# succinctlabs/sp1

Hardware: AMD Instinct MI355X
Metric: RISC-V cycles proved/sec (core shard prove): whole ShardProof of a full core shard of the reference's `fibonacci` guest, see config (higher is better)
Workload: dtype u32 (KoalaBear Montgomery words, exact integer arithmetic)

## Files before the change

### sp1_amd/csrc/gkr.hip

```cpp
#include <algorithm>
#include <array>
#include <chrono>
#include <cstring>
#include <memory>
#include <string>
#include <vector>

#include "device_ctx.hpp"
#include "host_par.hpp"

namespace sp1hip {
bool gkr_host_simd_available();
void gkr_host_round_sums(const uint32_t* tab, size_t stride, const uint32_t* eq, size_t eq_stride, size_t real_pairs, uint32_t out[6][4]);
void gkr_host_round_fold(const uint32_t* tab, uint32_t* out, size_t stride, size_t real_pairs, const uint32_t alpha[4]);
}
#include "round_sync.hpp"
#include "tensor_table.hpp"

namespace sp1hip {

void challenger_observe(sp1hip_challenger_t* ch, uint32_t x);
kb::Ext challenger_sample_ext(sp1hip_challenger_t* ch);
void challenger_restore(sp1hip_challenger_t* dst, const sp1hip_challenger_t* src);
void challenger_export(const sp1hip_challenger_t* ch, uint32_t* w34);
void challenger_import(sp1hip_challenger_t* ch, const uint32_t* w34);

namespace gkr {

using Ext = kb::Ext;
struct DeviceBuf : AsyncScratch {
    uint32_t* u32() const { return (uint32_t*)p; }
    Ext* ext() const { return (Ext*)p; }
};

__device__ __forceinline__ Ext ld_ext(const Ext* p, uint32_t i) {
    const q4_t v = gptr(reinterpret_cast<const q4_t*>(p))[i];
    return Ext{{v.x, v.y, v.z, v.w}};
}
__device__ __forceinline__ void st_ext(Ext* p, uint32_t i, const Ext& e) {
    const q4_t v = {e.c[0], e.c[1], e.c[2], e.c[3]};
    gptr(reinterpret_cast<q4_t*>(p))[i] = v;
}

__device__ __forceinline__ void st_ext_host(Ext* p, uint32_t i, const Ext& e) {
    uint32_t* w = reinterpret_cast<uint32_t*>(p + i);
#pragma unroll
    for (int k = 0; k < 4; k++) __hip_atomic_store(w + k, e.c[k], __ATOMIC_RELAXED, __HIP_MEMORY_SCOPE_SYSTEM);
}

__device__ __forceinline__ uint32_t wave_sum(uint32_t v) {
#pragma unroll
    for (int off = 32; off >= 1; off >>= 1) v = kb::add(v, __shfl_down(v, off, 64));
    return v;
}
template <int NS>
__device__ __forceinline__ void block_reduce_store(const Ext (&acc)[NS], uint32_t* out) {
    __shared__ uint32_t sm[4][4 * NS];
    const int lane = threadIdx.x & 63, wave = threadIdx.x >> 6;
#pragma unroll
    for (int s = 0; s < NS; s++)
#pragma unroll
        for (int k = 0; k < 4; k++) {
            const uint32_t w = wave_sum(acc[s].c[k]);
            if (lane == 0) sm[wave][4 * s + k] = w;
        }
    __syncthreads();
    if (threadIdx.x < 4 * NS) {
        uint32_t a = 0;
        for (int i = 0; i < 4; i++) a = kb::add(a, sm[i][threadIdx.x]);
        out[threadIdx.x] = a;
    }
}
template <int NS>
__global__ __launch_bounds__(256) void reduce_partials(const uint32_t* __restrict__ partials, uint32_t n, uint32_t* out) {
    Ext acc[NS];
#pragma unroll
    for (int s = 0; s < NS; s++) acc[s] = kb::ext_zero();
    for (uint32_t i = threadIdx.x; i < n; i += 256)
#pragma unroll
        for (int s = 0; s < NS; s++) {
            const uint32_t* q = partials + ((size_t)i * NS + s) * 4;
            acc[s] = kb::ext_add(acc[s], Ext{{q[0], q[1], q[2], q[3]}});
        }
    block_reduce_store<NS>(acc, out);
}

__device__ __forceinline__ uint32_t level_pos(uint32_t e, uint32_t len) {
    return (e | 511u) < len ? ((e & ~511u) | ((e & 7u) << 6) | ((e >> 3) & 63u)) : e;
}

struct IntDesc {
    const uint32_t* prog;
    const uint32_t* main;
    const uint32_t* prep;
    uint32_t rows;
    uint32_t* n_out;
    Ext* d_out;
};

// ... 442 lines not shown
            if (lane == 0) sm[wave][4 * c + k] = w;
        }
    }
    __syncthreads();
    if (threadIdx.x < 4 * OPEN_COLS) {
        const int c = threadIdx.x / 4;
        if (d.col0 + c < d.width) {
            uint32_t a = 0;
            for (int i = 0; i < 4; i++) a = kb::add(a, sm[i][threadIdx.x]);
            partials[((size_t)blockIdx.y * total_cols + d.out0 + c) * 4 + (threadIdx.x & 3)] = a;
        }
    }
}
__global__ __launch_bounds__(256) void open_sum_kernel(const uint32_t* __restrict__ partials, uint32_t n_chunks, uint32_t n_words, uint32_t* __restrict__ out) {
    __shared__ uint32_t sm[256];
    const uint32_t jl = threadIdx.x & 63u, cl = threadIdx.x >> 6, j = blockIdx.x * 64u + jl;
    uint32_t acc = 0;
    if (j < n_words)
        for (uint32_t c = cl; c < n_chunks; c += 4) acc = kb::add(acc, partials[(size_t)c * n_words + j]);
    sm[threadIdx.x] = acc;
    __syncthreads();
    if (cl == 0 && j < n_words) out[j] = kb::add(kb::add(sm[jl], sm[64 + jl]), kb::add(sm[128 + jl], sm[192 + jl]));
}

Ext operator+(const Ext& a, const Ext& b) { return kb::ext_add(a, b); }
Ext operator-(const Ext& a, const Ext& b) { return kb::ext_sub(a, b); }
Ext operator*(const Ext& a, const Ext& b) { return kb::ext_mul(a, b); }
Ext ext_c(uint32_t canonical) { return kb::ext_from_base(kb::to_monty(canonical)); }
int log2_ceil(uint64_t x) { int l = 0; while (((uint64_t)1 << l) < x) l++; return l; }

std::vector<Ext> partial_lagrange_host(const std::vector<Ext>& pt) {
    std::vector<Ext> ev{kb::ext_one()};
    for (const Ext& x : pt) {
        std::vector<Ext> nx(ev.size() * 2);
        for (size_t i = 0; i < ev.size(); i++) { const Ext pr = ev[i] * x; nx[2 * i] = ev[i] - pr; nx[2 * i + 1] = pr; }
        ev.swap(nx);
    }
    return ev;
}
Ext eval_mle_host(const std::vector<Ext>& vals, const std::vector<Ext>& pt) {
    const std::vector<Ext> eq = partial_lagrange_host(pt);
    Ext acc = kb::ext_zero();
    for (size_t i = 0; i < vals.size(); i++) acc = acc + eq[i] * vals[i];
    return acc;
}

using Poly4 = std::array<Ext, 4>;
Ext poly_eval(const Poly4& c, const Ext& x) { return ((c[3] * x + c[2]) * x + c[1]) * x + c[0]; }

Poly4 interpolate4(const Ext (&xs)[4], const Ext (&ys)[4]) {
    Poly4 res{kb::ext_zero(), kb::ext_zero(), kb::ext_zero(), kb::ext_zero()};
    Ext num[4][4], den[4];
    bool live[4];
    for (int i = 0; i < 4; i++) {
        live[i] = !kb::ext_eq(ys[i], kb::ext_zero());
        if (!live[i]) continue;
        den[i] = kb::ext_one();
        Ext cur[4] = {ys[i], kb::ext_zero(), kb::ext_zero(), kb::ext_zero()};
        int deg = 0;
        for (int j = 0; j < 4; j++) {
            if (j == i) continue;
            den[i] = den[i] * (xs[i] - xs[j]);
            Ext nxt[4] = {kb::ext_zero(), kb::ext_zero(), kb::ext_zero(), kb::ext_zero()};
            for (int k = 0; k <= deg; k++) { nxt[k + 1] = nxt[k + 1] + cur[k]; nxt[k] = nxt[k] - cur[k] * xs[j]; }
            deg++;
            for (int k = 0; k < 4; k++) cur[k] = nxt[k];
        }
        for (int k = 0; k < 4; k++) num[i][k] = cur[k];
    }
    Ext prefix[4], running = kb::ext_one();
    for (int i = 0; i < 4; i++) if (live[i]) { prefix[i] = running; running = running * den[i]; }
    Ext inv_all = kb::ext_inv(running);
    for (int i = 3; i >= 0; i--) {
        if (!live[i]) continue;
        const Ext inv = inv_all * prefix[i];
        inv_all = inv_all * den[i];
        for (int k = 0; k < 4; k++) res[k] = res[k] + num[i][k] * inv;
    }
    return res;
}

struct Bytes {
    std::vector<uint8_t> b;
    void u64(uint64_t v) { for (int i = 0; i < 8; i++) b.push_back((uint8_t)(v >> (8 * i))); }
    void felt(uint32_t m) { const uint32_t v = kb::from_monty(m); for (int i = 0; i < 4; i++) b.push_back((uint8_t)(v >> (8 * i))); }
    void ext(const Ext& e) { for (int k = 0; k < 4; k++) felt(e.c[k]); }
};

void observe_ext(sp1hip_challenger_t* ch, const Ext& e) { for (int k = 0; k < 4; k++) challenger_observe(ch, e.c[k]); }

int upload(DeviceBuf& buf, const void* src, size_t bytes, hipStream_t s, PinnedStage& stage) {
    SP1HIP_TRY(buf.alloc(std::max<size_t>(bytes, 16), s));
    return stage.upload(buf.p, src, bytes);
}

struct ChipInfo {
    std::string name;
    uint32_t rows, k, main_w, prep_w, int0;
    const uint32_t* d_main;
    const uint32_t* d_prep;
};

constexpr uint32_t MAX_TILES = 512;
uint32_t tiles_for(uint64_t threads) { return (uint32_t)std::min<uint64_t>(std::max<uint64_t>((threads + 255) / 256, 1), MAX_TILES); }
}
}

using namespace sp1hip;
using namespace sp1hip::gkr;

extern "C" {

int sp1hip_logup_gkr_prove(const sp1hip_gkr_chip_t* chips, int n_chips, int max_log_row_count, sp1hip_challenger_t* challenger,
                           uint8_t* h_proof, size_t* proof_len, sp1hip_stream_t stream) {
    SP1HIP_REQUIRE(chips && n_chips > 0 && challenger && proof_len, "bad argument");
    const int L = max_log_row_count;
    SP1HIP_REQUIRE(L >= 1 && L <= 30, "max_log_row_count out of range");
    hipStream_t s = S(stream);
    static const bool gkr_debug = env_flag("SP1HIP_GKR_DEBUG", false);
    auto t_last = std::chrono::steady_clock::now();
    auto mark = [&](const char* what) {
        if (!gkr_debug) return;
        const auto now = std::chrono::steady_clock::now();
        fprintf(stderr, "[sp1hip gkr] %-28s %8.3f ms\n", what, std::chrono::duration<double, std::milli>(now - t_last).count());
        t_last = now;
    };

    std::vector<ChipInfo> info(n_chips);
    struct ParsedInt { uint32_t is_send, kind; std::vector<uint32_t> mult; std::vector<std::vector<uint32_t>> values; };
    std::vector<ParsedInt> progs;
    size_t max_arity = 0, total_cols = 0;
    for (int c = 0; c < n_chips; c++) {
        const sp1hip_gkr_chip_t& ci = chips[c];
        SP1HIP_REQUIRE(ci.name && ci.interactions, "null chip field");
        SP1HIP_REQUIRE(ci.real_rows <= ((uint64_t)1 << L), "chip taller than 2^max_log_row_count");
        SP1HIP_REQUIRE(ci.real_rows == 0 || ci.main_width == 0 || ci.d_main, "null main trace");
        SP1HIP_REQUIRE(ci.real_rows == 0 || ci.prep_width == 0 || ci.d_prep, "null preprocessed trace");
        if (c) SP1HIP_REQUIRE(strcmp(chips[c - 1].name, ci.name) < 0, "chips must be sorted by name (BTreeSet order)");
        info[c] = ChipInfo{ci.name, (uint32_t)ci.real_rows, 0, ci.main_width, ci.prep_width, (uint32_t)progs.size(), ci.d_main, ci.d_prep};
        const uint32_t* p = ci.interactions;
        const uint32_t* end = p + ci.n_words;
        SP1HIP_REQUIRE(ci.n_words >= 1, "empty interaction program");
        const uint32_t ni = *p++;
        info[c].k = ni;
        auto vcol = [&](std::vector<uint32_t>& out) -> bool {
            if (p + 2 > end) return false;
            const uint32_t nt = p[0];
            if (p[1] >= kb::P || p + 2 + 3 * (size_t)nt > end) return false;
            out.push_back(nt);
            out.push_back(kb::to_monty(p[1]));
            p += 2;
            for (uint32_t t = 0; t < nt; t++, p += 3) {
                if (p[0] > 1 || p[2] >= kb::P) return false;
                if (p[1] >= (p[0] ? ci.main_width : ci.prep_width)) return false;
                out.push_back(p[0]); out.push_back(p[1]); out.push_back(kb::to_monty(p[2]));
            }
            return true;
        };
        for (uint32_t i = 0; i < ni; i++) {
            SP1HIP_REQUIRE(p + 3 <= end, "truncated interaction program");
            const uint32_t nv = p[2];
            SP1HIP_REQUIRE(p[0] <= 1 && p[1] < kb::P && nv < 4096, "bad interaction header");
            ParsedInt pi{p[0], p[1], {}, std::vector<std::vector<uint32_t>>(nv)};
            p += 3;
            SP1HIP_REQUIRE(vcol(pi.mult), "bad multiplicity column");
            for (uint32_t j = 0; j < nv; j++) SP1HIP_REQUIRE(vcol(pi.values[j]), "bad value column (index or weight out of range)");
            max_arity = std::max<size_t>(max_arity, nv + 1);
            progs.push_back(std::move(pi));
        }
        SP1HIP_REQUIRE(p == end, "trailing words in interaction program");
        total_cols += (size_t)ci.main_width + ci.prep_width;
    }
    const uint32_t K = (uint32_t)progs.size();
    SP1HIP_REQUIRE(K >= 1, "no interactions in the shard");
    const int niv = log2_ceil(K), beta_seed_dim = log2_ceil(max_arity);
    const uint32_t W = 1u << niv;

    size_t need = 2 * (8 + (size_t)2 * W * 16 + 24) + 8;
    for (int v = 1; v <= L - 1; v++) need += 64 + 8 + (size_t)(niv + v) * (8 + 64) + 16 + 8 + (size_t)(niv + v) * 16 + 16;
    need += 8 + (size_t)L * 16 + 8;
    for (int c = 0; c < n_chips; c++) {
        need += 8 + info[c].name.size() + 8 + (size_t)info[c].main_w * 16 + 16 + 1;
        if (info[c].prep_w) need += 8 + (size_t)info[c].prep_w * 16 + 16;
    }
    need += 4;
    if (!h_proof || *proof_len < need) {
        *proof_len = need;
        set_error("sp1hip_logup_gkr_prove: proof buffer too small, need %zu bytes", need);
        return SP1HIP_ERROR_BUFFER_TOO_SMALL;
    }

    const DeviceCtx* ctx;
    SP1HIP_TRY(get_device_ctx(&ctx));
    sp1hip_challenger_t* ch = nullptr;
    SP1HIP_TRY(sp1hip_challenger_clone(challenger, &ch));
    struct ChGuard { sp1hip_challenger_t* c; ~ChGuard() { sp1hip_challenger_free(c); } } guard{ch};

    uint32_t witness = 0;
    SP1HIP_TRY(sp1hip_challenger_grind(ch, 12, &witness, stream));
    const Ext alpha = challenger_sample_ext(ch);
    std::vector<Ext> beta_seed(beta_seed_dim);
    for (auto& b : beta_seed) b = challenger_sample_ext(ch);
    (void)challenger_sample_ext(ch);
    const std::vector<Ext> betas = partial_lagrange_host(beta_seed);

    auto rows_at = [&](uint32_t h, int l) -> uint32_t { return (uint32_t)(((uint64_t)h + (((uint64_t)1 << (L - l)) - 1)) >> (L - l)); };
    std::vector<uint32_t> int_chip(K);
    for (int c = 0; c < n_chips; c++) for (uint32_t i = 0; i < info[c].k; i++) int_chip[info[c].int0 + i] = c;
    std::vector<size_t> level_entries(L + 2, 0);
    for (int l = 1; l <= L; l++) for (uint32_t i = 0; i < K; i++) level_entries[l] += rows_at(info[int_chip[i]].rows, l);
    std::vector<DeviceBuf> lvN(L + 1), lvD(L + 1);
    for (int l = 1; l <= L; l++) {
        SP1HIP_TRY(lvN[l].alloc(std::max<size_t>(level_entries[l], 1) * (l == L ? 4 : 16), s));
        SP1HIP_TRY(lvD[l].alloc(std::max<size_t>(level_entries[l], 1) * 16, s));
    }
    std::vector<std::vector<size_t>> off(L + 1, std::vector<size_t>(K + 1, 0));
    for (int l = 1; l <= L; l++) for (uint32_t i = 0; i < K; i++) off[l][i + 1] = off[l][i] + rows_at(info[int_chip[i]].rows, l);
    auto n_ptr = [&](int l, uint32_t i) -> void* { return (char*)lvN[l].p + off[l][i] * (l == L ? 4 : 16); };
    auto d_ptr = [&](int l, uint32_t i) -> Ext* { return lvD[l].ext() + off[l][i]; };

    mark("parse + level buffers");
    const uint32_t FLAT_MAX_SLOTS = (uint32_t)env_uint("SP1HIP_GKR_FLAT_SLOTS", 65536);
    size_t n_passes_total = 0;
    for (int v = 1; v <= L - 1; v++) n_passes_total += (size_t)(v + 1) / 2 + 1;
    hipStream_t side = nullptr;
    hipEvent_t* side_ev = nullptr;
    SP1HIP_TRY(aux_stream_for(s, 2, &side, &side_ev));
    DeviceBuf d_all, d_flat;
    SP1HIP_TRY(d_all.alloc(std::max<size_t>(n_passes_total * K, 1) * sizeof(PassDesc), side));
    SP1HIP_TRY(d_flat.alloc((n_passes_total * (size_t)FLAT_MAX_SLOTS + 4) * sizeof(uint16_t), side));
    PinnedStage side_stage;
    SP1HIP_TRY(side_stage.init(side));
    PinnedStage stage;
    SP1HIP_TRY(stage.init(s));
    DeviceBuf d_progs, d_betas, d_descs;
    uint32_t max_rows = 0;
    bool fused_tree = false;
    std::vector<uint32_t> flat;
    std::vector<IntDesc> descs(K);
    {
        std::vector<size_t> poff(K);
        for (uint32_t i = 0; i < K; i++) {
            poff[i] = flat.size();
            const ParsedInt& pi = progs[i];
            Ext head = alpha + kb::ext_mul_base(betas[0], kb::to_monty(pi.kind));
            uint32_t live = 0;
            for (size_t j = 0; j < pi.values.size(); j++) {
                if (pi.values[j][0] == 0) head = head + kb::ext_mul_base(betas[1 + j], pi.values[j][1]);
                else live++;
            }
            flat.insert(flat.end(), {pi.is_send, live, head.c[0], head.c[1], head.c[2], head.c[3]});
            flat.insert(flat.end(), pi.mult.begin(), pi.mult.end());
            for (size_t j = 0; j < pi.values.size(); j++) {
                if (pi.values[j][0] == 0) continue;
                flat.push_back((uint32_t)(1 + j));
                flat.insert(flat.end(), pi.values[j].begin(), pi.values[j].end());
            }
        }
        SP1HIP_TRY(upload(d_progs, flat.data(), flat.size() * 4, s, stage));
        SP1HIP_TRY(upload(d_betas, betas.data(), betas.size() * 16, s, stage));
        for (uint32_t i = 0; i < K; i++) {
            const ChipInfo& c = info[int_chip[i]];
            descs[i] = IntDesc{d_progs.u32() + poff[i], c.d_main, c.d_prep, c.rows, (uint32_t*)n_ptr(L, i), d_ptr(L, i)};
            max_rows = std::max(max_rows, c.rows);
        }
        fused_tree = L >= 3 && env_flag("SP1HIP_GKR_FUSED", true);
        if (fused_tree) {
            std::vector<FirstDesc> fdescs(K);
            for (uint32_t i = 0; i < K; i++)
                fdescs[i] = FirstDesc{descs[i].prog, descs[i].main, descs[i].prep, descs[i].rows, descs[i].n_out, descs[i].d_out,
                                      (Ext*)n_ptr(L - 1, i), d_ptr(L - 1, i), (Ext*)n_ptr(L - 2, i), d_ptr(L - 2, i)};
            SP1HIP_TRY(upload(d_descs, fdescs.data(), fdescs.size() * sizeof(FirstDesc), s, stage));
            if (max_rows) {
                ScopedTimer t("gkr_first_layer", s);
                hipLaunchKernelGGL(first_layers_kernel, dim3(tiles_for((max_rows + 3) / 4), K), dim3(256), 0, s, (const FirstDesc*)d_descs.p,
                                   (const Ext*)d_betas.p);
                SP1HIP_LAUNCH_CHECK();
            }
        } else {
            SP1HIP_TRY(upload(d_descs, descs.data(), descs.size() * sizeof(IntDesc), s, stage));
            if (max_rows) {
                ScopedTimer t("gkr_first_layer", s);
                hipLaunchKernelGGL(first_layer_kernel, dim3(tiles_for(max_rows), K), dim3(256), 0, s, (const IntDesc*)d_descs.p,
                                   (const Ext*)d_betas.p);
                SP1HIP_LAUNCH_CHECK();
            }
        }
    }
    mark("first layer enqueued");
    DeviceBuf d_trans, d_trans2;
    {
        const int top = fused_tree ? L - 2 : L;
        std::vector<Trans2Desc> t2;
        std::vector<TransDesc> t1;
        std::vector<uint32_t> t2_mr, t1_mr;
        std::vector<int> t1_level;
        int l = top;
        if (fused_tree)
            for (; l >= 3; l -= 2) {
                uint32_t mr = 0;
                for (uint32_t i = 0; i < K; i++) {
                    const uint32_t rin = rows_at(info[int_chip[i]].rows, l);
                    t2.push_back(Trans2Desc{(const Ext*)n_ptr(l, i), d_ptr(l, i), (Ext*)n_ptr(l - 1, i), d_ptr(l - 1, i), (Ext*)n_ptr(l - 2, i), d_ptr(l - 2, i), rin});
                    mr = std::max(mr, (rin + 3) / 4);
                }
                t2_mr.push_back(mr);
            }
        for (; l >= 2; l--) {
            uint32_t mr = 0;
            for (uint32_t i = 0; i < K; i++) {
                const uint32_t rin = rows_at(info[int_chip[i]].rows, l);
                t1.push_back(TransDesc{n_ptr(l, i), d_ptr(l, i), (Ext*)n_ptr(l - 1, i), d_ptr(l - 1, i), rin});
                mr = std::max(mr, (rin + 1) / 2);
            }
            t1_mr.push_back(mr);
            t1_level.push_back(l);
        }
        if (!t2.empty()) SP1HIP_TRY(upload(d_trans2, t2.data(), t2.size() * sizeof(Trans2Desc), s, stage));
        if (!t1.empty()) SP1HIP_TRY(upload(d_trans, t1.data(), t1.size() * sizeof(TransDesc), s, stage));
        for (size_t k = 0; k < t2_mr.size(); k++) {
            if (!t2_mr[k]) continue;
            ScopedTimer t("gkr_transition", s);
            hipLaunchKernelGGL(transition2_kernel, dim3(tiles_for(t2_mr[k]), K), dim3(256), 0, s, (const Trans2Desc*)d_trans2.p + k * K);
            SP1HIP_LAUNCH_CHECK();
        }
        for (size_t k = 0; k < t1_mr.size(); k++) {
            if (!t1_mr[k]) continue;
            const TransDesc* d_t = (const TransDesc*)d_trans.p + k * K;
            ScopedTimer t("gkr_transition", s);
            if (t1_level[k] == L) hipLaunchKernelGGL(transition_kernel<true>, dim3(tiles_for(t1_mr[k]), K), dim3(256), 0, s, d_t);
            else hipLaunchKernelGGL(transition_kernel<false>, dim3(tiles_for(t1_mr[k]), K), dim3(256), 0, s, d_t);
            SP1HIP_LAUNCH_CHECK();
        }
    }
    mark("tree enqueued");
    Mailbox mb;
    SP1HIP_TRY(mb.init(s));
    struct RoundOut { Ext n0, n1, d0, d1; std::vector<Poly4> polys; Ext claimed_sum, eval; std::vector<Ext> point; };
    std::vector<RoundOut> rounds;
    DeviceBuf d_eq_int, d_T, d_TL, d_partials, scratch[2];
// ... 9 lines not shown
    std::vector<uint16_t> flat_index;
    constexpr uint32_t TARGET_TILES = 2048;
    std::vector<PassDesc> all_descs;
    all_descs.reserve(n_passes_total * K);
    const bool direct_final = (size_t)K * 16 + 4 <= MAILBOX_WORDS;
    Ext* const host_rows = reinterpret_cast<Ext*>(mb.h_slot + 4);
    for (int v = 1; v <= L - 1; v++) {
        std::vector<uint32_t> rows_in(K);
        for (uint32_t i = 0; i < K; i++) rows_in[i] = (rows_at(info[int_chip[i]].rows, v + 1) + 1) / 2;
        int cur = 0, t = v, fv = 0, pass = 0;
        std::vector<size_t> so_prev, so_next;
        for (;;) {
            const int sv = std::min(2, t - fv);
            const bool first = pass <= 1;
            if (fv > 0) { so_next.assign(K + 1, 0); for (uint32_t i = 0; i < K; i++) so_next[i + 1] = so_next[i] + ((rows_in[i] + (1u << fv) - 1) >> fv); }
            uint64_t total_slots = 0;
            auto slots_of = [&](uint32_t rin) -> uint32_t { const uint32_t ro = (rin + (1u << fv) - 1) >> fv; return ((ro + (1u << sv) - 1) >> sv) << sv; };
            for (uint32_t i = 0; i < K; i++) total_slots += slots_of(rows_in[i]);
            const bool flat = total_slots <= FLAT_MAX_SLOTS && K <= 65536;
            const uint32_t tile_size = flat ? 1u : (uint32_t)std::max<uint64_t>(256, ((total_slots + TARGET_TILES - 1) / TARGET_TILES + 255) / 256 * 256);
            const size_t flat_off = flat_index.size();
            all_descs.resize(all_descs.size() + K);
            PassDesc* out = all_descs.data() + all_descs.size() - K;
            uint32_t tile0 = 0;
            for (uint32_t i = 0; i < K; i++) {
                PassDesc& d = out[i];
                d = PassDesc{};
                d.rows_in = rows_in[i]; d.eq_int_index = i;
                if (first) { d.src[0] = n_ptr(v + 1, i); d.src[1] = d_ptr(v + 1, i); d.rows_x = rows_at(info[int_chip[i]].rows, v + 1); }
                else for (int w = 0; w < 4; w++) d.src[w] = scratch_ptr(cur ^ 1, i, w, so_prev);
                if (fv > 0) for (int w = 0; w < 4; w++)
                    d.dst[w] = (sv == 0 && direct_final) ? host_rows + 4 * so_next[i] + (size_t)w * (so_next[i + 1] - so_next[i]) : scratch_ptr(cur, i, w, so_next);
                d.tile0 = tile0;
                const uint32_t n_tiles = (slots_of(rows_in[i]) + tile_size - 1) / tile_size;
                if (flat) flat_index.insert(flat_index.end(), n_tiles, (uint16_t)i);
                tile0 += n_tiles;
            }
            if (flat) shapes.push_back(PassShape{fv, sv, first, std::max<uint32_t>((tile0 + 255) / 256, 1), tile_size, tile0, flat_off, true});
            else shapes.push_back(PassShape{fv, sv, first, std::max<uint32_t>(tile0, 1), tile_size, tile0, 0, false});
            if (fv > 0) { for (uint32_t i = 0; i < K; i++) rows_in[i] = (rows_in[i] + (1u << fv) - 1) >> fv; so_prev = so_next; cur ^= 1; }
            t -= fv;
            pass++;
            if (sv == 0) break;
            fv = sv;
        }
    }
    {
        uint32_t max_tiles = 1;
        for (auto& sh : shapes) max_tiles = std::max(max_tiles, sh.tiles);
        SP1HIP_TRY(d_partials.alloc((size_t)max_tiles * 160, s));
    }
    mark("pass descriptors planned");
    SP1HIP_REQUIRE(all_descs.size() == n_passes_total * K, "internal error: pass count");
    SP1HIP_TRY(side_stage.upload(d_all.p, all_descs.data(), all_descs.size() * sizeof(PassDesc)));
    if (flat_index.empty()) flat_index.push_back(0);
    flat_index.resize((flat_index.size() + 1) / 2 * 2);
    SP1HIP_REQUIRE(flat_index.size() * sizeof(uint16_t) <= d_flat.n, "internal error: flat index size");
    SP1HIP_TRY(side_stage.upload(d_flat.p, flat_index.data(), flat_index.size() * sizeof(uint16_t)));
    SP1HIP_HIP(hipEventRecord(side_ev[1], side));
    SP1HIP_HIP(hipStreamWaitEvent(s, side_ev[1], 0));
    mark("pass descriptors uploaded");
    std::vector<Ext> out_n(2 * (size_t)W, kb::ext_zero()), out_d(2 * (size_t)W, kb::ext_one());
    {
        std::vector<Ext> hn(std::max<size_t>(level_entries[1], 1)), hd(std::max<size_t>(level_entries[1], 1));
        if (L >= 2) {
            SP1HIP_TRY(mb.fetch(lvN[1].p, level_entries[1] * 4, hn.data()));
        } else {
            std::vector<uint32_t> hb(std::max<size_t>(level_entries[1], 1));
            SP1HIP_TRY(mb.fetch(lvN[1].p, level_entries[1], hb.data()));
            for (size_t e = 0; e < level_entries[1]; e++) hn[e] = kb::ext_from_base(hb[e]);
        }
        SP1HIP_TRY(mb.fetch(lvD[1].p, level_entries[1] * 4, hd.data()));
        for (uint32_t i = 0; i < K; i++)
            for (uint32_t r = 0; r < rows_at(info[int_chip[i]].rows, 1); r++) { out_n[2 * i + r] = hn[off[1][i] + r]; out_d[2 * i + r] = hd[off[1][i] + r]; }
    }
    mark("circuit output fetched");
    challenger_observe(ch, kb::to_monty(2 * W));
    for (auto& e : out_n) observe_ext(ch, e);
    challenger_observe(ch, kb::to_monty(2 * W));
    for (auto& e : out_d) observe_ext(ch, e);
    std::vector<Ext> eval_point(niv + 1);
    for (auto& z : eval_point) z = challenger_sample_ext(ch);
    Ext num_eval = eval_mle_host(out_n, eval_point), den_eval = eval_mle_host(out_d, eval_point);

    size_t launch_idx = 0;
    RoundSyncHost rsync;
    SP1HIP_TRY(rsync.init(s));
    const Ext one = kb::ext_one(), zero = kb::ext_zero(), inv8 = kb::ext_inv(ext_c(8)), inv2 = kb::ext_inv(ext_c(2)), four = ext_c(4);
    uint32_t h_sums[40];
    auto eq_times_quadratic = [&](const Ext& scale, const Ext& pt, const Ext (&q)[3]) -> Poly4 {
        const Ext e0 = scale * (one - pt), e1 = scale * (pt + pt - one);
        return Poly4{e0 * q[0], e0 * q[1] + e1 * q[0], e0 * q[2] + e1 * q[1], e1 * q[2]};
    };
    auto quadratic = [&](const Ext& g0, const Ext& g1, const Ext& gi, Ext (&q)[3]) { q[0] = g0; q[1] = g1 - g0 - gi; q[2] = gi; };
    auto eval_quadratic = [&](const Ext (&q)[3], const Ext& x) -> Ext { return (q[2] * x + q[1]) * x + q[0]; };

    const bool simd = gkr_host_simd_available();
    HostPar::Scope par;
    par.park();
    double dbg_rows = 0, dbg_int = 0, dbg_head = 0;
    auto dbg_t = std::chrono::steady_clock::now();
    auto dbg_pass_t = dbg_t;
    double dbg_wait = 0, dbg_host = 0, dbg_launch = 0;
    int dbg_passes = 0;
    bool dbg_pass_pending = false;
    for (int v = 1; v <= L - 1; v++) {
        if (gkr_debug) dbg_t = std::chrono::steady_clock::now();
        const Ext lambda = challenger_sample_ext(ch);
        RoundOut ro;
        Ext claim = num_eval * lambda + den_eval;
        ro.claimed_sum = claim;
        const std::vector<Ext> int_point(eval_point.begin(), eval_point.begin() + niv), row_point(eval_point.begin() + niv, eval_point.end());
        SP1HIP_REQUIRE(niv <= 32 && v <= 32, "point too long");
        {
            PointArg pi{}, pa{};
            for (int j = 0; j < niv; j++) pi.c[j] = int_point[j];
            for (int j = 0; j < v; j++) pa.c[j] = row_point[j];
            const uint32_t full_blocks = (W + 255) / 256, prefix_blocks = ((2u << v) + 255) / 256;
            hipLaunchKernelGGL(eq_layer_tables_kernel, dim3(full_blocks + prefix_blocks), dim3(256), 0, s, pi, niv, d_eq_int.ext(), full_blocks, pa, v,
                               lambda, d_T.ext(), d_TL.ext());
            SP1HIP_LAUNCH_CHECK();
        }
        std::vector<std::vector<Ext>> eq_tabs(niv + 1);
        std::vector<std::vector<uint32_t>> eq_soa(niv + 1);
        auto eq_plane_stride = [](int m) { return ((((size_t)1 << m) + 15) / 16) * 16 + 16; };
        bool eq_tabs_built = false;
        auto build_eq_tabs = [&]() {
            if (eq_tabs_built) return;
            eq_tabs_built = true;
            eq_tabs[0] = {one};
            for (int m = 0; m < niv; m++) {
                const std::vector<Ext>& ev = eq_tabs[m];
                std::vector<Ext>& nx = eq_tabs[m + 1];
                nx.resize(ev.size() * 2);
                const Ext x = int_point[m];
                for (size_t i = 0; i < ev.size(); i++) { const Ext pr = ev[i] * x; nx[2 * i] = ev[i] - pr; nx[2 * i + 1] = pr; }
            }
            if (simd)
                for (int m = 1; m <= niv; m++) {
                    const size_t es = eq_plane_stride(m);
                    eq_soa[m].assign(4 * es, 0u);
                    for (size_t i = 0; i < eq_tabs[m].size(); i++)
                        for (int k = 0; k < 4; k++) eq_soa[m][(size_t)k * es + i] = eq_tabs[m][i].c[k];
                }
        };
        auto T_of = [&](int t) -> const Ext* { return d_T.ext() + (((size_t)1 << t) - 1); };
        auto TL_of = [&](int t) -> const Ext* { return d_TL.ext() + (((size_t)1 << t) - 1); };

        std::vector<Ext> alphas;
        Ext PA = one;
        Ext a0 = zero, a1 = zero;
        int t = v;
        size_t final_rows_total = 0;
        auto launch_pass = [&](size_t idx, int t_after, const Ext& c0, const Ext& c1) -> int {
            const PassShape shape = shapes[idx];
            const PassDesc* d_descs = (const PassDesc*)d_all.p + idx * K;
            const int fv = shape.fv, sv = shape.sv;
            const FlatArgs fa{(const uint16_t*)d_flat.p + shape.flat_off, shape.total_slots};
            const bool nbase = shape.first && v + 1 == L;
            const bool publish_rows = sv == 0 && direct_final;
            if (publish_rows) { rsync.pending = true; mb.pending = true; }
            const RoundSync rs = sv > 0 ? rsync.next() : publish_rows ? RoundSync{rsync.d_counter, (volatile uint32_t*)mb.h_slot} : RoundSync{};
            const Ext* Tp = sv > 0 ? T_of(t_after - sv) : (const Ext*)nullptr;
            const Ext* TLp = sv > 0 ? TL_of(t_after - sv) : (const Ext*)nullptr;
            ScopedTimer tm(fv == 0 ? "gkr_pass_sum" : sv == 0 ? "gkr_pass_fold" : "gkr_pass_fold_sum", s);
#define SP1HIP_GKR_PASS(FV, SV, F, NB, FL) hipLaunchKernelGGL((gkr_pass<FV, SV, F, NB, FL>), dim3(shape.tiles), dim3(256), 0, s, d_descs, (const Ext*)d_eq_int.p, Tp, TLp, c0, c1, d_partials.u32(), rs, publish_rows ? mb.seq + 1 : rsync.seq, K, shape.tile_size, fa)
// ... 165 lines not shown
                        for (int k = 0; k < 4; k++) soa[side ^ 1][(size_t)(4 * w + k) * soa_stride + real_pairs] = (w & 1) && k == 0 ? one.c[0] : 0u;
            } else
            par.run(real_pairs, 48, [&](int, size_t kb0, size_t ke) {
                for (size_t k = kb0; k < ke; k++) {
                    o0[k] = n0[2 * k] + alpha_r * (n0[2 * k + 1] - n0[2 * k]); o1[k] = d0[2 * k] + alpha_r * (d0[2 * k + 1] - d0[2 * k]);
                    o2[k] = n1[2 * k] + alpha_r * (n1[2 * k + 1] - n1[2 * k]); o3[k] = d1[2 * k] + alpha_r * (d1[2 * k + 1] - d1[2 * k]);
                }
            });
            if (!simd && real_pairs < half) { o0[real_pairs] = kb::ext_zero(); o1[real_pairs] = one; o2[real_pairs] = kb::ext_zero(); o3[real_pairs] = one; }
            real = real_pairs;
            side ^= 1;
        }
        Ext fin_n0 = (*tab[side][0])[0], fin_d0 = (*tab[side][1])[0], fin_n1 = (*tab[side][2])[0], fin_d1 = (*tab[side][3])[0];
        if (simd) {
            Ext* f[4] = {&fin_n0, &fin_d0, &fin_n1, &fin_d1};
            for (int w = 0; w < 4; w++)
                for (int k = 0; k < 4; k++) f[w]->c[k] = soa[side][(size_t)(4 * w + k) * soa_stride];
        }
        if (gkr_debug) { const auto now = std::chrono::steady_clock::now(); dbg_int += std::chrono::duration<double, std::milli>(now - dbg_t).count(); dbg_t = now; }
        ro.eval = claim;
        ro.point.assign(alphas.rbegin(), alphas.rend());
        ro.n0 = fin_n0; ro.d0 = fin_d0; ro.n1 = fin_n1; ro.d1 = fin_d1;
        observe_ext(ch, ro.n0); observe_ext(ch, ro.n1); observe_ext(ch, ro.d0); observe_ext(ch, ro.d1);
        eval_point = ro.point;
        const Ext lc = challenger_sample_ext(ch);
        num_eval = ro.n0 + (ro.n1 - ro.n0) * lc;
        den_eval = ro.d0 + (ro.d1 - ro.d0) * lc;
        eval_point.push_back(lc);
        rounds.push_back(std::move(ro));
        par.park();
    }

    if (gkr_debug) fprintf(stderr, "[sp1hip gkr]   of which row-variable rounds %.3f ms, interaction-variable rounds (host) %.3f ms\n", dbg_rows, dbg_int);
    if (gkr_debug) fprintf(stderr, "[sp1hip gkr]   %d hand-overs inside the layers: waiting for the sums %.3f ms, closed forms + transcript %.3f ms, launch calls %.3f ms\n",
                           dbg_passes, dbg_wait, dbg_host, dbg_launch);
    (void)dbg_head;
    mark("all layers");
    const std::vector<Ext> trace_point(eval_point.end() - L, eval_point.end());
    std::vector<Ext> openings(std::max<size_t>(total_cols, 1), kb::ext_zero());
    if (total_cols) {
        DeviceBuf d_eq, d_od, d_part, d_res;
        SP1HIP_TRY(d_eq.alloc(((size_t)16) << L, s));
        SP1HIP_TRY(sp1hip_partial_lagrange(reinterpret_cast<const sp1hip_ext_t*>(trace_point.data()), L, d_eq.u32(), stream));
        std::vector<OpenDesc> od;
        uint32_t out0 = 0, max_rows_open = 0;
        for (int c = 0; c < n_chips; c++) {
            for (uint32_t g = 0; g < info[c].main_w; g += OPEN_COLS) od.push_back(OpenDesc{info[c].d_main, info[c].rows, info[c].main_w, g, out0 + g});
            out0 += info[c].main_w;
            for (uint32_t g = 0; g < info[c].prep_w; g += OPEN_COLS) od.push_back(OpenDesc{info[c].d_prep, info[c].rows, info[c].prep_w, g, out0 + g});
            out0 += info[c].prep_w;
            max_rows_open = std::max(max_rows_open, info[c].rows);
        }
        const uint32_t chunks = std::max<uint32_t>((max_rows_open + OPEN_ROWS - 1) / OPEN_ROWS, 1);
        SP1HIP_TRY(upload(d_od, od.data(), od.size() * sizeof(OpenDesc), s, stage));
        SP1HIP_TRY(d_part.alloc((size_t)chunks * total_cols * 16, s));
        SP1HIP_TRY(d_res.alloc(total_cols * 16, s));
        SP1HIP_HIP(hipMemsetAsync(d_part.p, 0, (size_t)chunks * total_cols * 16, s));
        ScopedTimer t("gkr_openings", s);
        hipLaunchKernelGGL(open_columns_kernel, dim3((uint32_t)od.size(), chunks), dim3(256), 0, s, (const OpenDesc*)d_od.p, d_eq.u32(),
                           1u << L, d_part.u32(), (uint32_t)total_cols);
        SP1HIP_LAUNCH_CHECK();
        hipLaunchKernelGGL(open_sum_kernel, dim3(((uint32_t)total_cols * 4 + 63) / 64), dim3(256), 0, s, d_part.u32(), chunks,
                           (uint32_t)total_cols * 4, d_res.u32());
        SP1HIP_LAUNCH_CHECK();
        SP1HIP_TRY(mb.fetch(d_res.p, total_cols * 4, openings.data()));
    }
    challenger_observe(ch, kb::to_monty((uint32_t)n_chips));
    {
        size_t o = 0;
        for (int c = 0; c < n_chips; c++) {
            const Ext* main = openings.data() + o;
            const Ext* prep = main + info[c].main_w;
            if (info[c].prep_w) {
                challenger_observe(ch, kb::to_monty(info[c].prep_w));
                for (uint32_t k = 0; k < info[c].prep_w; k++) observe_ext(ch, prep[k]);
            }
            challenger_observe(ch, kb::to_monty(info[c].main_w));
            for (uint32_t k = 0; k < info[c].main_w; k++) observe_ext(ch, main[k]);
            o += info[c].main_w + info[c].prep_w;
        }
    }

    mark("openings");
    Bytes w;
    for (const std::vector<Ext>* vv : {&out_n, &out_d}) {
        w.u64(vv->size());
        for (auto& e : *vv) w.ext(e);
        w.u64(2); w.u64(vv->size()); w.u64(1);
    }
    w.u64(rounds.size());
    for (auto& r : rounds) {
        w.ext(r.n0); w.ext(r.n1); w.ext(r.d0); w.ext(r.d1);
        w.u64(r.polys.size());
        for (auto& p : r.polys) { w.u64(4); for (auto& c : p) w.ext(c); }
        w.ext(r.claimed_sum);
        w.u64(r.point.size());
        for (auto& x : r.point) w.ext(x);
        w.ext(r.eval);
    }
    w.u64(trace_point.size());
    for (auto& x : trace_point) w.ext(x);
    w.u64(n_chips);
    {
        size_t o = 0;
        for (int c = 0; c < n_chips; c++) {
            w.u64(info[c].name.size());
            for (char chr : info[c].name) w.b.push_back((uint8_t)chr);
            w.u64(info[c].main_w);
            for (uint32_t k = 0; k < info[c].main_w; k++) w.ext(openings[o + k]);
            w.u64(1); w.u64(info[c].main_w);
            w.b.push_back(info[c].prep_w ? 1 : 0);
            if (info[c].prep_w) {
                w.u64(info[c].prep_w);
                for (uint32_t k = 0; k < info[c].prep_w; k++) w.ext(openings[o + info[c].main_w + k]);
                w.u64(1); w.u64(info[c].prep_w);
            }
            o += info[c].main_w + info[c].prep_w;
        }
    }
    w.felt(witness);
    if (w.b.size() != need) {
        set_error("internal error: GKR proof size %zu != expected %zu", w.b.size(), need);
        return SP1HIP_ERROR_RUNTIME;
    }
    memcpy(h_proof, w.b.data(), w.b.size());
    *proof_len = w.b.size();
    challenger_restore(challenger, ch);
    return SP1HIP_SUCCESS;
}

}
```

### sp1_amd/csrc/jagged.hip

```cpp
#include <cstring>
#include <memory>
#include <vector>

#include <algorithm>
#include <array>

#include "device_ctx.hpp"
#include "jagged_host.hpp"
#include "round_sync.hpp"
#include "stacked_data.hpp"
#include "tensor_table.hpp"

namespace sp1hip {

struct DeviceBuf : AsyncScratch {
    uint32_t* u32() const { return (uint32_t*)p; }
};

void challenger_observe(sp1hip_challenger_t* ch, uint32_t x);
kb::Ext challenger_sample_ext(sp1hip_challenger_t* ch);
void challenger_restore(sp1hip_challenger_t* dst, const sp1hip_challenger_t* src);

using Ext = kb::Ext;

// ... 746 lines not shown
                           half, (Ext*)d_state.p, (Ext*)d_inter.p, sc.tail());
        SP1HIP_LAUNCH_CHECK();
        Ext y0, yh;
        SP1HIP_TRY(sc.finish(nb, &y0, &yh));
        poly = interpolate(y0, yh + yh + yh + yh, claim - y0);
        proof->polys.push_back(poly);
        alpha = observe_and_sample(ch, poly);
        alphas.push_back(alpha);
        claim = poly_eval(poly, alpha);
    }
    std::vector<Ext> B((size_t)D * 2 * 16);
    for (int layer = 0; layer < D; layer++)
        for (int cb = 0; cb < 2; cb++)
            for (int e = 0; e < 16; e++) {
                const Ext a0 = mats[((size_t)layer * 4 + cb * 2 + 0) * 16 + e], a1 = mats[((size_t)layer * 4 + cb * 2 + 1) * 16 + e];
                B[((size_t)layer * 2 + cb) * 16 + e] = a0 + alphas[layer] * (a1 - a0);
            }
    DeviceBuf d_B, d_suffix2;
    SP1HIP_TRY(upload(d_B, B.data(), B.size() * 16, s, sc.stage));
    SP1HIP_TRY(d_suffix2.alloc((size_t)D * n * 64, s));
    hipLaunchKernelGGL(je_suffix_kernel<false>, dim3(nb), dim3(256), 0, s, C, (const Ext*)d_B.p, D, (Ext*)d_suffix2.p, sc.tail());
    SP1HIP_LAUNCH_CHECK();
    Ext W[4] = {kb::ext_one(), kb::ext_zero(), kb::ext_zero(), kb::ext_zero()};
    for (int rp = 0; rp < D; rp++) {
        Ext V[8];
        for (int b = 0; b < 2; b++)
            for (int k = 0; k < 4; k++) {
                Ext acc = kb::ext_zero();
                for (int m = 0; m < 4; m++) acc = acc + W[m] * B[((size_t)rp * 2 + b) * 16 + 4 * m + k];
                V[4 * b + k] = acc;
            }
        JeV Varg;
        memcpy(Varg.v, V, sizeof V);
        hipLaunchKernelGGL(je_phase2_round, dim3(nb), dim3(256), 0, s, C, (const Ext*)d_suffix2.p, D, rp, alpha, half,
                           Varg, (Ext*)d_inter.p, sc.tail());
        SP1HIP_LAUNCH_CHECK();
        Ext y0, yh;
        SP1HIP_TRY(sc.finish(nb, &y0, &yh));
        poly = interpolate(y0, yh + yh + yh + yh, claim - y0);
        proof->polys.push_back(poly);
        alpha = observe_and_sample(ch, poly);
        alphas.push_back(alpha);
        claim = poly_eval(poly, alpha);
        for (int k = 0; k < 4; k++) W[k] = V[k] + alpha * (V[4 + k] - V[k]);
    }
    (void)dim;
    proof->point.assign(alphas.rbegin(), alphas.rend());
    proof->eval = claim;
    return SP1HIP_SUCCESS;
}

}

size_t jagged_proof_size_with(size_t opening_bytes, size_t commitment_bytes, const std::vector<uint32_t>& round_widths,
                              const std::vector<size_t>& tables_per_round, uint64_t total_area) {
    const int n_rounds = (int)round_widths.size();
    const int log_m = log2_ceil(total_area), D = log_m + 1;
    size_t need = opening_bytes;
    need += 8;
    for (uint32_t w : round_widths) need += 8 + (size_t)w * 16 + 16;
    need += 8 + (size_t)log_m * (8 + 48) + 16 + 8 + (size_t)log_m * 16 + 16;
    need += 8 + (size_t)2 * D * (8 + 48) + 16 + 8 + (size_t)2 * D * 16 + 16;
    need += 8;
    for (size_t t : tables_per_round) need += 8 + t * 16;
    need += 8 + (size_t)n_rounds * commitment_bytes + 16 + 8 + 8;
    return need;
}

size_t jagged_proof_size(int lsh, const std::vector<uint32_t>& round_widths, const std::vector<size_t>& tables_per_round,
                         uint64_t total_area, sp1hip_fri_config_t config) {
    return jagged_proof_size_with(sp1hip_basefold_proof_size(lsh, round_widths.data(), (int)round_widths.size(), config), 32, round_widths,
                                  tables_per_round, total_area);
}

int jagged_prove_with(JaggedBackend& be, const sp1hip_ext_t* h_z_row, int max_log_row_count, StackedCore* const* rounds, int n_rounds,
                      const sp1hip_ext_t* h_claims, const size_t* claims_per_round, sp1hip_fri_config_t config, uint8_t* h_proof,
                      size_t* proof_len, sp1hip_stream_t stream) {
    SP1HIP_REQUIRE(h_z_row && rounds && n_rounds > 0 && n_rounds <= 8 && claims_per_round && proof_len, "bad argument");
    SP1HIP_REQUIRE(max_log_row_count >= 0 && max_log_row_count <= 30, "max_log_row_count out of range");
    hipStream_t s = S(stream);
    const bool jg_timing = env_flag("SP1HIP_JG_TIMING", false);
    std::chrono::steady_clock::time_point jg_t[7];
    jg_t[0] = std::chrono::steady_clock::now();
    struct StageMarks {
        bool open = false;
        void next(const char* name) { if (open) roctx_pop(); roctx_push(name); open = true; }
        ~StageMarks() { if (open) roctx_pop(); }
    } marks;
    marks.next("jagged_setup");
    SP1HIP_REQUIRE(rounds[0], "null round");
    const int lsh = rounds[0]->log_stacking_height;
    SP1HIP_REQUIRE(lsh >= 1, "log_stacking_height must be at least 1");
    uint64_t total_cols = 0, total_area = 0, n_claims = 0;
    std::vector<uint32_t> round_widths;
    for (int r = 0; r < n_rounds; r++) {
        const StackedCore* d = rounds[r];
        SP1HIP_REQUIRE(d && d->jagged, "round data did not come from a jagged commit");
        if (d->stream != s) rounds[r]->foreign_use = true;
        SP1HIP_REQUIRE(d->log_stacking_height == lsh && d->max_log_row_count == max_log_row_count, "rounds disagree on parameters");
        SP1HIP_REQUIRE(d->area > 0, "a commitment round without any table data cannot be opened");
        uint64_t expect = 0;
        for (size_t t = 0; t + 2 < d->column_counts.size(); t++) expect += d->column_counts[t];
        SP1HIP_REQUIRE(claims_per_round[r] == expect, "claims_per_round does not match the committed tables");
        for (uint64_t c : d->column_counts) total_cols += c;
        total_area += d->padded;
        n_claims += claims_per_round[r];
        round_widths.push_back((uint32_t)(d->padded >> lsh));
    }
    SP1HIP_REQUIRE(h_claims || n_claims == 0, "null claims");
    SP1HIP_REQUIRE(total_area < ((uint64_t)1 << 30), "dense area must stay below 2^30 (jagged verifier bound)");
    const int log_m = log2_ceil(total_area);
    SP1HIP_REQUIRE(log_m >= lsh, "internal: area smaller than one stacked column");
    const int num_col_variables = log2_ceil(total_cols);
    std::vector<size_t> tables_per_round;
    for (int r = 0; r < n_rounds; r++) tables_per_round.push_back(rounds[r]->row_counts.size());
    const size_t need = jagged_proof_size_with(be.opening_size(lsh, round_widths.data(), n_rounds, config), be.commitment_bytes(),
                                               round_widths, tables_per_round, total_area);
    if (!h_proof || *proof_len < need) {
        *proof_len = need;
        set_error("%s: proof buffer too small, need %zu bytes", be.entry_point(), need);
        return SP1HIP_ERROR_BUFFER_TOO_SMALL;
    }
    const DeviceCtx* ctx;
    SP1HIP_TRY(get_device_ctx(&ctx));

    JaggedBackend& ch = be;
    SP1HIP_TRY(be.begin());

    std::vector<Ext> z_row(max_log_row_count), z_col(num_col_variables);
    memcpy(z_row.data(), h_z_row, (size_t)max_log_row_count * 16);
    for (auto& z : z_col) z = ch.sample_ext();

    std::vector<Ext> column_claims;
    {
        size_t off = 0;
        for (int r = 0; r < n_rounds; r++) {
            for (size_t i = 0; i < claims_per_round[r]; i++) { Ext e; memcpy(&e, &h_claims[off + i], 16); column_claims.push_back(e); }
            off += claims_per_round[r];
            column_claims.insert(column_claims.end(), rounds[r]->padding_column_count, kb::ext_zero());
        }
    }
    SP1HIP_REQUIRE(column_claims.size() == total_cols, "internal: column claim count");
    const Ext sumcheck_claim = eval_ext_mle_host(column_claims, z_col);

    std::vector<uint32_t> prefix;
    {
        uint64_t acc = 0;
        for (int r = 0; r < n_rounds; r++)
            for (size_t t = 0; t < rounds[r]->row_counts.size(); t++)
                for (uint64_t c = 0; c < rounds[r]->column_counts[t]; c++) { prefix.push_back((uint32_t)acc); acc += rounds[r]->row_counts[t]; }
        prefix.push_back((uint32_t)acc);
        SP1HIP_REQUIRE(acc == total_area, "internal: prefix sums do not cover the dense area");
    }
    const uint32_t ncols = (uint32_t)prefix.size() - 1;
    const std::vector<Ext> col_eq = partial_lagrange_host(z_col);

    Scratch sc;
    SP1HIP_TRY(sc.init(s));
    DeviceBuf d_prefix, d_col_eq, d_row_eq;
    SP1HIP_TRY(upload(d_prefix, prefix.data(), prefix.size() * 4, s, sc.stage));
    SP1HIP_TRY(upload(d_col_eq, col_eq.data(), col_eq.size() * 16, s, sc.stage));
    SP1HIP_TRY(d_row_eq.alloc(((size_t)16) << max_log_row_count, s));
    SP1HIP_TRY(sp1hip_partial_lagrange(h_z_row, max_log_row_count, d_row_eq.u32(), stream));
    JgSegs segs{};
    segs.n = n_rounds;
    {
        uint64_t start = 0;
        for (int r = 0; r < n_rounds; r++) {
            segs.s[r] = JgSeg{(const uint32_t*)rounds[r]->d_dense, (uint32_t)start, (uint32_t)rounds[r]->padded};
            start += rounds[r]->padded;
        }
        segs.total = (uint32_t)start;
    }
    const JgJ J{d_prefix.u32(), ncols, (const Ext*)d_col_eq.p, d_row_eq.u32(), 1u << max_log_row_count};
    const uint32_t T = segs.total;

    marks.next("jagged_sumcheck");
    Sumcheck sumcheck;
    sumcheck.claimed_sum = sumcheck_claim;
    std::vector<Ext> alphas;
    Ext claim = sumcheck_claim, alpha = kb::ext_zero(), q_eval = kb::ext_zero(), j_eval = kb::ext_zero();
    std::array<Ext, 3> poly{};
    DeviceBuf tabs[4];
    const uint32_t n1 = (T + 1) / 2;
    const bool factored_enabled = env_flag("SP1HIP_JAGGED_FACTORED", true);
    int rf = 0;
    {
        uint32_t g = T;
        for (uint32_t pfx : prefix) g |= pfx;
        rf = g ? __builtin_ctz(g) : 0;
        rf = std::min(rf, std::min(log_m - 2, max_log_row_count - 1));
        if (!factored_enabled) rf = 0;
        if (rf < 2) rf = 0;
    }
    bool j_materialised = rf == 0;
    if (rf == 0) {
        SP1HIP_TRY(tabs[1].alloc((size_t)std::max<uint32_t>(n1, 1) * 16, s));
        SP1HIP_TRY(tabs[3].alloc((size_t)std::max<uint32_t>((n1 + 1) / 2, 1) * 16, s));
    }
    DeviceBuf row_eq_lv[2], d_prefix_lv;
    const uint32_t* row_eq_cur = d_row_eq.u32();
    uint32_t row_len_cur = 1u << max_log_row_count;
    if (rf) {
        SP1HIP_TRY(row_eq_lv[0].alloc(((size_t)16) << (max_log_row_count - 1), s));
        SP1HIP_TRY(row_eq_lv[1].alloc(((size_t)16) << (max_log_row_count - 1), s));
        SP1HIP_TRY(d_prefix_lv.alloc(prefix.size() * 4 * (size_t)(rf + 1), s));
        std::vector<uint32_t> all_lv(prefix.size() * (size_t)(rf + 1));
        for (int lv = 0; lv <= rf; lv++)
            for (size_t c = 0; c < prefix.size(); c++) all_lv[(size_t)lv * prefix.size() + c] = prefix[c] >> lv;
        SP1HIP_TRY(sc.stage.upload(d_prefix_lv.p, all_lv.data(), all_lv.size() * 4));
    }
    auto level_J = [&](int lv, const Ext& a_prev, JgJ* out) -> int {
        uint32_t* dst = row_eq_lv[lv & 1].u32();
        hipLaunchKernelGGL(jg_fold_row_eq, dim3((row_len_cur / 2 + 255) / 256), dim3(256), 0, s, row_eq_cur, row_len_cur, a_prev, dst);
        SP1HIP_LAUNCH_CHECK();
        row_eq_cur = dst;
        row_len_cur >>= 1;
        uint32_t* d_pl = d_prefix_lv.u32() + (size_t)lv * prefix.size();
        *out = JgJ{d_pl, ncols, (const Ext*)d_col_eq.p, row_eq_cur, row_len_cur};
        return SP1HIP_SUCCESS;
    };
    std::vector<JgTab> tabs0;
    uint32_t n_tiles0 = 0, n_tiles1 = 0, n_tiles2 = 0;
    bool tables_mult4 = false;
    bool skip_level1 = false;
    std::vector<std::pair<uint64_t, uint64_t>> zero_tails;
    DeviceBuf d_tabs0, d_col_eq3;
    {
        uint32_t g = T;
        for (uint32_t pfx : prefix) g |= pfx;
        if ((g & 1u) == 0 && factored_enabled) {
            uint64_t seg_start = 0;
            uint32_t col = 0;
            for (int r = 0; r < n_rounds; r++) {
                const StackedCore* d = rounds[r];
                uint64_t off = 0;
                const size_t n_real = d->row_counts.size() - 2;
                for (size_t t = 0; t < d->row_counts.size(); t++) {
                    const uint32_t h = (uint32_t)d->row_counts[t], w = (uint32_t)d->column_counts[t];
                    if (t < n_real && h && w) {
                        for (uint32_t c_lo = 0; c_lo < w; c_lo += JG_COL_SLICE) {
                            const uint32_t wc = std::min(JG_COL_SLICE, w - c_lo);
                            const uint64_t o = off + (uint64_t)c_lo * h;
                            tabs0.push_back(JgTab{(const uint32_t*)d->d_dense + o, h, col + c_lo, wc, n_tiles0, (uint32_t)(seg_start + o), n_tiles1, n_tiles2});
                            n_tiles0 += (h / 2 + JG_TAB_PAIRS - 1) / JG_TAB_PAIRS;
                            n_tiles1 += ((h + 3) / 4 + JG_TAB_PAIRS - 1) / JG_TAB_PAIRS;
                            n_tiles2 += ((h + 7) / 8 + JG_TAB_PAIRS - 1) / JG_TAB_PAIRS;
                        }
                    }
                    if (t == n_real) zero_tails.push_back({seg_start + off, seg_start + d->padded});
                    off += (uint64_t)h * w;
                    col += w;
                }
                seg_start += d->padded;
            }
            if (!tabs0.empty()) {
                SP1HIP_TRY(upload(d_tabs0, tabs0.data(), tabs0.size() * sizeof(JgTab), s, sc.stage));
                tables_mult4 = (g & 3u) == 0;
                skip_level1 = (g & 7u) == 0 && rf >= 2 && log_m >= 4;
                std::vector<Ext> col_eq3(col_eq.size());
                for (size_t c = 0; c < col_eq.size(); c++)
                    for (int q = 0; q < 4; q++) col_eq3[c].c[q] = kb::add(kb::dbl(col_eq[c].c[q]), col_eq[c].c[q]);
                SP1HIP_TRY(upload(d_col_eq3, col_eq3.data(), col_eq3.size() * 16, s, sc.stage));
            }
        }
    }
    SP1HIP_TRY(tabs[0].alloc((size_t)std::max<uint32_t>(skip_level1 ? (T + 7) / 8 : n1, 1) * 16, s));
    SP1HIP_TRY(tabs[2].alloc((size_t)std::max<uint32_t>((n1 + 1) / 2, 1) * 16, s));
    uint32_t n_live = T;
    int cur = 0;
    jg_t[1] = std::chrono::steady_clock::now();
    const bool lookahead01 = skip_level1 && !tabs0.empty() && log_m >= 2 && env_flag("SP1HIP_JAGGED_LOOKAHEAD", true);
    for (int round = 0; round < log_m; round++) {
        uint32_t nb;
        if (round == 0 && lookahead01) {
            {
                ScopedTimer t("jagged_round0_sum", s);
                nb = Scratch::blocks_for((uint64_t)n_tiles1 * 256);
                hipLaunchKernelGGL(jg_round01_tables, dim3(nb), dim3(256), 0, s, (const JgTab*)d_tabs0.p, (uint32_t)tabs0.size(), n_tiles1, J,
                                   sc.tail());
                SP1HIP_LAUNCH_CHECK();
            }
            Ext S[8];
            SP1HIP_TRY(sc.finish8(S));
            const Ext y0 = S[0] + S[1], h0 = S[2] + S[3];
            poly = interpolate(y0, h0, claim - y0);
            sumcheck.polys.push_back(poly);
            alpha = observe_and_sample(ch, poly);
            alphas.push_back(alpha);
            claim = poly_eval(poly, alpha);
            {
                JgJ J1;
                SP1HIP_TRY(level_J(1, alpha, &J1));
            }
            const Ext a0 = alpha;
            const Ext c0 = S[0], c2 = (S[0] + S[4]) + (S[0] + S[4]) - S[2], c1 = S[4] - c0 - c2;
            const Ext d0 = S[5], d2 = S[7], d1 = S[6] - d0 - d2;
            const Ext y1 = c0 + (c1 + c2 * a0) * a0, h1 = d0 + (d1 + d2 * a0) * a0;
            poly = interpolate(y1, h1, claim - y1);
            sumcheck.polys.push_back(poly);
            alpha = observe_and_sample(ch, poly);
            alphas.push_back(alpha);
            claim = poly_eval(poly, alpha);
            n_live = (n_live + 1) / 2;
            cur = 0;
            round = 1;
            continue;
        }
        if (round == 0) {
            ScopedTimer t("jagged_round0_sum", s);
            if (!tabs0.empty()) {
                nb = Scratch::blocks_for((uint64_t)n_tiles0 * 256);
                hipLaunchKernelGGL(jg_round0_tables, dim3(nb), dim3(256), 0, s, (const JgTab*)d_tabs0.p, (uint32_t)tabs0.size(), n_tiles0, J,
                                   sc.tail());
            } else {
                nb = Scratch::blocks_for((T / 2 + JG_ITERS - 1) / JG_ITERS);
                hipLaunchKernelGGL(jg_round0_sum, dim3(nb), dim3(256), 0, s, segs, J, T / 2, sc.tail());
            }
        } else if (round == 1) {
            ScopedTimer t("jagged_fold0_sum", s);
            const uint32_t n_out = (n_live + 1) / 2;
            nb = Scratch::blocks_for(((n_out + 1) / 2 + JG_ITERS - 1) / JG_ITERS);
            if (rf) {
                JgJ J1;
                SP1HIP_TRY(level_J(1, alpha, &J1));
                if (skip_level1) {
                    nb = Scratch::blocks_for((uint64_t)n_tiles1 * 256);
                    hipLaunchKernelGGL((jg_fold_tables<1, false>), dim3(nb), dim3(256), 0, s, (const JgTab*)d_tabs0.p, (uint32_t)tabs0.size(),
                                       n_tiles1, J1, (const Ext*)d_col_eq3.p, alpha, alpha, (Ext*)nullptr, sc.tail());
                } else if (tables_mult4) {
                    for (auto& z : zero_tails)
                        if (z.second > z.first) SP1HIP_HIP(hipMemsetAsync((Ext*)tabs[0].p + z.first / 2, 0, (size_t)((z.second - z.first) / 2) * 16, s));
                    nb = Scratch::blocks_for((uint64_t)n_tiles1 * 256);
                    hipLaunchKernelGGL((jg_fold_tables<1, true>), dim3(nb), dim3(256), 0, s, (const JgTab*)d_tabs0.p, (uint32_t)tabs0.size(),
                                       n_tiles1, J1, (const Ext*)d_col_eq3.p, alpha, alpha, (Ext*)tabs[0].p, sc.tail());
                } else {
                    hipLaunchKernelGGL(jg_fold0_sum<false>, dim3(nb), dim3(256), 0, s, segs, J, alpha, n_out, (Ext*)tabs[0].p, (Ext*)nullptr,
                                       sc.tail());
                }
            } else {
                hipLaunchKernelGGL(jg_fold0_sum<true>, dim3(nb), dim3(256), 0, s, segs, J, alpha, n_out, (Ext*)tabs[0].p, (Ext*)tabs[1].p,
                                   sc.tail());
            }
            n_live = n_out;
            cur = 0;
        } else {
            ScopedTimer t("jagged_fold_sum", s);
            const uint32_t n_out = (n_live + 1) / 2;
            const int nxt = cur ^ 2;
            if (round == 2 && skip_level1) {
                JgJ Jl;
                SP1HIP_TRY(level_J(2, alpha, &Jl));
                for (auto& z : zero_tails)
                    if (z.second > z.first) SP1HIP_HIP(hipMemsetAsync((Ext*)tabs[nxt].p + z.first / 4, 0, (size_t)((z.second - z.first) / 4) * 16, s));
                nb = Scratch::blocks_for((uint64_t)n_tiles2 * 256);
                hipLaunchKernelGGL((jg_fold_tables<2, true>), dim3(nb), dim3(256), 0, s, (const JgTab*)d_tabs0.p, (uint32_t)tabs0.size(),
                                   n_tiles2, Jl, (const Ext*)d_col_eq3.p, alphas[0], alpha, (Ext*)tabs[nxt].p, sc.tail());
            } else if (round <= rf) {
                JgJ Jl;
                SP1HIP_TRY(level_J(round, alpha, &Jl));
                nb = Scratch::blocks_for(((n_out + 1) / 2 + JG_ITERS - 1) / JG_ITERS);
                hipLaunchKernelGGL(jg_foldf_sum, dim3(nb), dim3(256), 0, s, (const Ext*)tabs[cur].p, n_live, Jl, alpha, n_out,
                                   (Ext*)tabs[nxt].p, sc.tail());
            } else {
                nb = Scratch::blocks_for((n_out + 1) / 2);
                if (!j_materialised) {
                    const JgJ Jp{d_prefix_lv.u32() + (size_t)(round - 1) * prefix.size(), ncols, (const Ext*)d_col_eq.p, row_eq_cur, row_len_cur};
                    SP1HIP_TRY(tabs[cur + 1].alloc((size_t)std::max<uint32_t>((n_out + 1) / 2, 1) * 16, s));
                    SP1HIP_TRY(tabs[nxt + 1].alloc((size_t)std::max<uint32_t>(n_out, 1) * 16, s));
                    j_materialised = true;
                    hipLaunchKernelGGL(jg_fold_sum_fj, dim3(nb), dim3(256), 0, s, (const Ext*)tabs[cur].p, Jp, n_live, alpha, n_out,
                                       (Ext*)tabs[nxt].p, (Ext*)tabs[nxt + 1].p, sc.tail());
                } else {
                    hipLaunchKernelGGL(jg_fold_sum, dim3(nb), dim3(256), 0, s, (const Ext*)tabs[cur].p, (const Ext*)tabs[cur + 1].p, n_live,
                                       alpha, n_out, (Ext*)tabs[nxt].p, (Ext*)tabs[nxt + 1].p, sc.tail());
                }
            }
            n_live = n_out;
            cur = nxt;
        }
        SP1HIP_LAUNCH_CHECK();
        Ext y0, h4;
        SP1HIP_TRY(sc.finish(nb, &y0, &h4));
        poly = interpolate(y0, h4, claim - y0);
        sumcheck.polys.push_back(poly);
        alpha = observe_and_sample(ch, poly);
        alphas.push_back(alpha);
        claim = poly_eval(poly, alpha);
    }
    sumcheck.point.assign(alphas.rbegin(), alphas.rend());
    sumcheck.eval = claim;
    if (log_m == 0) {
        SP1HIP_REQUIRE(false, "degenerate dense area");
    } else if (log_m == 1) {
        uint32_t hq[2];
        SP1HIP_TRY(sc.mb.fetch(rounds[0]->d_dense, 2, hq));
        q_eval = kb::ext_from_base(hq[0]) + kb::ext_mul_base(alpha, kb::sub(hq[1], hq[0]));
    } else {
        Ext hq[2] = {kb::ext_zero(), kb::ext_zero()}, hj[2] = {kb::ext_zero(), kb::ext_zero()};
        SP1HIP_TRY(sc.mb.fetch(tabs[cur].p, (size_t)n_live * 4, hq));
        SP1HIP_TRY(sc.mb.fetch(tabs[cur + 1].p, (size_t)n_live * 4, hj));
        q_eval = hq[0] + alpha * (hq[1] - hq[0]);
        j_eval = hj[0] + alpha * (hj[1] - hj[0]);
    }
    (void)j_eval;
    const std::vector<Ext>& final_point = sumcheck.point;

    jg_t[2] = std::chrono::steady_clock::now();
    marks.next("jagged_eval");
    Sumcheck jagged_eval;
    SP1HIP_TRY(jagged_eval_prove(prefix, log_m, z_row, z_col, final_point, ch, sc, &jagged_eval));
    jg_t[3] = std::chrono::steady_clock::now();
    marks.next("stacked_basefold_open");

    for (int k = 0; k < 4; k++) ch.observe(q_eval.c[k]);
    const std::vector<Ext> stack_point(final_point.end() - lsh, final_point.end());
    DeviceBuf d_eq, d_evals;
    SP1HIP_TRY(d_eq.alloc(((size_t)16) << lsh, s));
    SP1HIP_TRY(sp1hip_partial_lagrange(reinterpret_cast<const sp1hip_ext_t*>(stack_point.data()), lsh, d_eq.u32(), stream));
    std::vector<std::vector<Ext>> batch_evals(n_rounds);
    std::vector<Ext> flat_claims;
    SP1HIP_TRY(d_evals.alloc((size_t)(*std::max_element(round_widths.begin(), round_widths.end())) * 16, s));
    for (int r = 0; r < n_rounds; r++) {
        const uint32_t w = round_widths[r];
        batch_evals[r].resize(w);
        ScopedTimer t("jagged_batch_evals", s);
        SP1HIP_TRY(sp1hip_mle_eval_columns(rounds[r]->batches.data(), (int)rounds[r]->batches.size(), lsh, d_eq.u32(), d_evals.u32(), stream));
        SP1HIP_TRY(sc.mb.fetch(d_evals.p, (size_t)w * 4, batch_evals[r].data()));
        flat_claims.insert(flat_claims.end(), batch_evals[r].begin(), batch_evals[r].end());
    }
    for (auto& e : flat_claims) for (int k = 0; k < 4; k++) ch.observe(e.c[k]);
    jg_t[4] = std::chrono::steady_clock::now();
    size_t bf_len = need;
    SP1HIP_TRY(be.open(reinterpret_cast<const sp1hip_ext_t*>(stack_point.data()), lsh,
                       reinterpret_cast<const sp1hip_ext_t*>(flat_claims.data()), flat_claims.size(), config, h_proof, &bf_len, stream));

    jg_t[5] = std::chrono::steady_clock::now();
    Bytes w;
    w.p = h_proof;
    w.cap = need;
    w.n = bf_len;
    w.u64(n_rounds);
    for (auto& ev : batch_evals) { w.u64(ev.size()); for (auto& e : ev) w.ext(e); w.u64(1); w.u64(ev.size()); }
    sumcheck.write(w);
    jagged_eval.write(w);
    w.u64(n_rounds);
    for (int r = 0; r < n_rounds; r++) {
        w.u64(rounds[r]->row_counts.size());
        for (size_t t = 0; t < rounds[r]->row_counts.size(); t++) { w.u64(rounds[r]->row_counts[t]); w.u64(rounds[r]->column_counts[t]); }
    }
    w.u64(n_rounds);
    for (int r = 0; r < n_rounds; r++) {
        uint8_t c[64];
        be.write_commitment(r, c);
        w.raw(c, be.commitment_bytes());
    }
    w.ext(q_eval);
    w.u64(max_log_row_count);
    w.u64(log_m);
    if (w.overflow || w.n != need) {
        set_error("internal error: jagged proof size %zu != expected %zu", w.n, need);
        return SP1HIP_ERROR_RUNTIME;
    }
    *proof_len = w.n;
    be.accept();
    if (jg_timing) {
        jg_t[6] = std::chrono::steady_clock::now();
        const auto ms = [&](int a, int b) { return std::chrono::duration<double, std::milli>(jg_t[b] - jg_t[a]).count(); };
        fprintf(stderr, "[sp1hip jagged] set-up %.3f ms | %d sumcheck rounds %.3f | jagged-eval %.3f | column evaluations %.3f | BaseFold %.3f | proof bytes %.3f\n",
                ms(0, 1), log_m, ms(1, 2), ms(2, 3), ms(3, 4), ms(4, 5), ms(5, 6));
    }
    return SP1HIP_SUCCESS;
}

namespace {
struct InnerJaggedBackend final : JaggedBackend {
    sp1hip_challenger_t* caller;
    sp1hip_challenger_t* work = nullptr;
    sp1hip_stacked_data_t* const* rounds;
    int n_rounds;
    InnerJaggedBackend(sp1hip_challenger_t* c, sp1hip_stacked_data_t* const* r, int n) : caller(c), rounds(r), n_rounds(n) {}
    ~InnerJaggedBackend() override { sp1hip_challenger_free(work); }
    const char* entry_point() const override { return "sp1hip_jagged_prove"; }
    int begin() override { return sp1hip_challenger_clone(caller, &work); }
    void observe(uint32_t monty) override { challenger_observe(work, monty); }
    Ext sample_ext() override { return challenger_sample_ext(work); }
    void accept() override { challenger_restore(caller, work); }
    size_t opening_size(int dim, const uint32_t* widths, int n, sp1hip_fri_config_t config) const override {
        return sp1hip_basefold_proof_size(dim, widths, n, config);
    }
    int open(const sp1hip_ext_t* h_point, int dim, const sp1hip_ext_t* h_claims, size_t n_claims, sp1hip_fri_config_t config,
             uint8_t* h_proof, size_t* len, sp1hip_stream_t stream) override {
        std::vector<sp1hip_basefold_data_t*> bf;
        for (int r = 0; r < n_rounds; r++) bf.push_back(rounds[r]->basefold);
        return sp1hip_basefold_prove(h_point, dim, bf.data(), n_rounds, h_claims, n_claims, config, work, h_proof, len, stream);
    }
    size_t commitment_bytes() const override { return 32; }
    void write_commitment(int round, uint8_t* dst) const override {
        for (int k = 0; k < 8; k++) { const uint32_t v = kb::from_monty(rounds[round]->commit[k]); memcpy(dst + 4 * k, &v, 4); }
    }
};
}
}

using namespace sp1hip;

extern "C" {

int sp1hip_jagged_prove(const sp1hip_ext_t* h_z_row, int max_log_row_count, sp1hip_stacked_data_t* const* rounds, int n_rounds,
                        const sp1hip_ext_t* h_claims, const size_t* claims_per_round, sp1hip_fri_config_t config,
                        sp1hip_challenger_t* challenger, uint8_t* h_proof, size_t* proof_len, sp1hip_stream_t stream) {
    SP1HIP_REQUIRE(rounds && n_rounds > 0 && n_rounds <= 8 && challenger, "bad argument");
    std::vector<StackedCore*> cores(rounds, rounds + n_rounds);
    InnerJaggedBackend be(challenger, rounds, n_rounds);
    return jagged_prove_with(be, h_z_row, max_log_row_count, cores.data(), n_rounds, h_claims, claims_per_round, config, h_proof,
                             proof_len, stream);
}

}
```

### sp1_amd/csrc/shard.hip

```cpp
#include <chrono>
#include <cstring>
#include <memory>
#include <string>
#include <mutex>
#include <unordered_map>
#include <vector>

#include "device_ctx.hpp"
#include "stacked_data.hpp"

namespace sp1hip {
void challenger_observe(sp1hip_challenger_t* ch, uint32_t x);
kb::Ext challenger_sample_ext(sp1hip_challenger_t* ch);
void challenger_restore(sp1hip_challenger_t* dst, const sp1hip_challenger_t* src);
size_t jagged_proof_size(int lsh, const std::vector<uint32_t>& round_widths, const std::vector<size_t>& tables_per_round,
                         uint64_t total_area, sp1hip_fri_config_t config);

namespace {

struct Reader {
    const uint8_t* p;
    size_t n, o = 0;
    uint64_t u64() { uint64_t v = 0; for (int i = 0; i < 8; i++) v |= (uint64_t)p[o + i] << (8 * i); o += 8; return v; }
    uint32_t canonical() { uint32_t v = 0; for (int i = 0; i < 4; i++) v |= (uint32_t)p[o + i] << (8 * i); o += 4; return v; }
    kb::Ext ext() { kb::Ext e; for (int k = 0; k < 4; k++) e.c[k] = kb::to_monty(canonical()); return e; }
    void skip(size_t k) { o += k; }
};

void put_u64(std::vector<uint8_t>& b, uint64_t v) { for (int i = 0; i < 8; i++) b.push_back((uint8_t)(v >> (8 * i))); }
void put_felt(std::vector<uint8_t>& b, uint32_t monty) { const uint32_t v = kb::from_monty(monty); for (int i = 0; i < 4; i++) b.push_back((uint8_t)(v >> (8 * i))); }

}
}

using namespace sp1hip;

extern "C" {

int sp1hip_prove_shard(const sp1hip_shard_chip_t* chips, int n_chips, const uint32_t* h_publics, int n_publics,
                       sp1hip_stacked_data_t* preprocessed, sp1hip_shard_params_t params, sp1hip_challenger_t* challenger,
                       uint8_t* h_proof, size_t* proof_len, sp1hip_stream_t stream) {
    SP1HIP_REQUIRE(chips && n_chips > 0 && preprocessed && challenger && proof_len, "bad argument");
    SP1HIP_REQUIRE(h_publics || n_publics == 0, "null public values");
    ActiveProver active;
    const auto sh_entry = std::chrono::steady_clock::now();
    uint64_t miss_n0 = 0, miss_b0 = 0;
    arena_miss_stats(&miss_n0, &miss_b0);
    const int L = params.max_log_row_count, lsh = params.log_stacking_height;
    SP1HIP_REQUIRE(preprocessed->jagged && preprocessed->max_log_row_count == L && preprocessed->log_stacking_height == lsh,
                   "the preprocessed round was committed with different parameters");
    hipStream_t s = S(stream);

    std::vector<sp1hip_gkr_chip_t> gk(n_chips);
    std::vector<sp1hip_zc_chip_t> zc(n_chips);
    std::vector<sp1hip_table_t> tables(n_chips);
    uint64_t main_area = 0;
    size_t total_w = 0, prep_cols = 0, opened_bytes = 8;
    for (int c = 0; c < n_chips; c++) {
        const sp1hip_shard_chip_t& ci = chips[c];
        SP1HIP_REQUIRE(ci.name && ci.program && ci.interactions, "null chip field");
        SP1HIP_REQUIRE(ci.main_width > 0, "a chip needs at least one main column");
        gk[c] = sp1hip_gkr_chip_t{ci.name, ci.interactions, ci.n_words, ci.main_width, ci.prep_width, ci.d_main, ci.d_prep, ci.real_rows};
        zc[c] = sp1hip_zc_chip_t{ci.program, ci.n_instr, ci.main_width, ci.prep_width, ci.num_constraints, ci.d_main, ci.d_prep, ci.real_rows};
        tables[c] = sp1hip_table_t{ci.d_main, ci.real_rows, ci.main_width};
        main_area += ci.real_rows * (uint64_t)ci.main_width;
        total_w += ci.main_width + ci.prep_width;
        prep_cols += ci.prep_width;
        opened_bytes += 8 + strlen(ci.name) + 8 + (size_t)ci.prep_width * 16 + 8 + (size_t)ci.main_width * 16 + 8 + (size_t)(L + 1) * 4;
    }
    SP1HIP_REQUIRE(prep_cols > 0, "a shard needs at least one preprocessed column (two commitment rounds)");
    SP1HIP_REQUIRE(main_area > 0, "empty shard");
    uint64_t shape_sig = 0xcbf29ce484222325ull;
    {
        auto mix = [&](uint64_t v) { shape_sig = (shape_sig ^ v) * 0x100000001b3ull; };
        mix((uint64_t)n_chips); mix((uint64_t)L); mix((uint64_t)lsh); mix((uint64_t)params.fri.log_blowup); mix((uint64_t)params.fri.num_queries);
        for (int c = 0; c < n_chips; c++) { mix(chips[c].real_rows); mix((uint64_t)chips[c].main_width << 32 | (uint32_t)chips[c].n_instr); }
    }

    size_t gkr_size = 0, zc_size = 0;
    uint64_t size_sig = shape_sig;
    for (int c = 0; c < n_chips; c++) {
        size_sig = (size_sig ^ ((uint64_t)chips[c].n_words << 32 | chips[c].num_constraints)) * 0x100000001b3ull;
        size_sig = (size_sig ^ ((uint64_t)strlen(chips[c].name) << 32 | chips[c].prep_width)) * 0x100000001b3ull;
    }
    size_sig = (size_sig ^ (uint64_t)n_publics) * 0x100000001b3ull;
    static std::mutex size_mutex;
    static std::unordered_map<uint64_t, std::pair<size_t, size_t>> size_cache;
    bool have_sizes = false;
    {
        std::lock_guard<std::mutex> lk(size_mutex);
        auto it = size_cache.find(size_sig);
        if (it != size_cache.end()) { gkr_size = it->second.first; zc_size = it->second.second; have_sizes = true; }
    }
    if (!have_sizes) {
        int st = sp1hip_logup_gkr_prove(gk.data(), n_chips, L, challenger, nullptr, &gkr_size, stream);
        if (st != SP1HIP_ERROR_BUFFER_TOO_SMALL) return st == SP1HIP_SUCCESS ? SP1HIP_ERROR_RUNTIME : st;
        std::vector<sp1hip_ext_t> dummy(std::max<size_t>({total_w, (size_t)L, 1}));
        st = sp1hip_zerocheck_prove(zc.data(), n_chips, L, dummy.data(), dummy.data(), dummy[0], dummy[0], h_publics, n_publics,
                                    challenger, nullptr, &zc_size, stream);
        if (st != SP1HIP_ERROR_BUFFER_TOO_SMALL) return st == SP1HIP_SUCCESS ? SP1HIP_ERROR_RUNTIME : st;
        std::lock_guard<std::mutex> lk(size_mutex);
        if (size_cache.size() > 4096) size_cache.clear();
        size_cache[size_sig] = {gkr_size, zc_size};
    }
    const uint64_t H = (uint64_t)1 << lsh;
    const uint64_t main_padded = std::max<uint64_t>((main_area + H - 1) / H, 1) * H;
    const std::vector<uint32_t> round_widths{(uint32_t)(preprocessed->padded >> lsh), (uint32_t)(main_padded >> lsh)};
    const std::vector<size_t> tables_per_round{preprocessed->row_counts.size(), (size_t)n_chips + 2};
    const size_t jag_size = jagged_proof_size(lsh, round_widths, tables_per_round, preprocessed->padded + main_padded, params.fri);
    const size_t zc_sumcheck_size = zc_size - (8 + (size_t)n_chips * 8 + total_w * 16);
    const size_t need = 8 + (size_t)n_publics * 4 + 32 + gkr_size + zc_sumcheck_size + opened_bytes + jag_size;
    if (!h_proof || *proof_len < need) {
        *proof_len = need;
        set_error("sp1hip_prove_shard: proof buffer too small, need %zu bytes", need);
        return SP1HIP_ERROR_BUFFER_TOO_SMALL;
    }

    const bool sh_timing = env_flag("SP1HIP_SHARD_TIMING", false);
    std::chrono::steady_clock::time_point sh_t[6];
    sh_t[0] = std::chrono::steady_clock::now();
    RoctxRange proof_range("sp1hip_prove_shard");
    struct StageMarks {
        hipStream_t s;
        bool open = false;
        int idx = -1;
        void close() { if (idx >= 0) timer_end(idx, s); idx = -1; if (open) roctx_pop(); open = false; set_stage_note(""); }
        void next(const char* name) {
            close();
            roctx_push(name);
            set_stage_note(name);
            open = true;
            if (timers_on()) { char buf[64]; snprintf(buf, sizeof buf, "stage_%s", name); idx = timer_begin(buf, s); }
        }
        ~StageMarks() { close(); }
    } marks{S(stream)};
    WaitPlan wait_plan(shape_sig);
    marks.next("commit");
    sp1hip_challenger_t* ch = nullptr;
    SP1HIP_TRY(sp1hip_challenger_clone(challenger, &ch));
    struct ChGuard { sp1hip_challenger_t* c; ~ChGuard() { sp1hip_challenger_free(c); } } guard{ch};

    for (int i = 0; i < n_publics; i++) {
        SP1HIP_REQUIRE(h_publics[i] < kb::P, "public value not reduced");
        challenger_observe(ch, h_publics[i]);
    }
    uint32_t main_commit[8];
    sp1hip_stacked_data_t* main_data = nullptr;
    SP1HIP_TRY(sp1hip_jagged_commit(tables.data(), n_chips, L, lsh, params.batch_size, params.fri.log_blowup, main_commit, &main_data, stream));
    std::unique_ptr<sp1hip_stacked_data_s> main_guard(main_data);
    for (int k = 0; k < 8; k++) challenger_observe(ch, main_commit[k]);
    challenger_observe(ch, kb::to_monty((uint32_t)n_chips));
    for (int c = 0; c < n_chips; c++) {
        challenger_observe(ch, kb::to_monty((uint32_t)chips[c].real_rows));
        const size_t nl = strlen(chips[c].name);
        challenger_observe(ch, kb::to_monty((uint32_t)nl));
        for (size_t b = 0; b < nl; b++) challenger_observe(ch, kb::to_monty((uint8_t)chips[c].name[b]));
    }

    sh_t[1] = std::chrono::steady_clock::now();
    marks.next("logup_gkr");
    std::vector<uint8_t> gkr_blob(gkr_size);
    size_t glen = gkr_size;
    SP1HIP_TRY(sp1hip_logup_gkr_prove(gk.data(), n_chips, L, ch, gkr_blob.data(), &glen, stream));
    std::vector<kb::Ext> zeta(L), openings;
    {
        Reader r{gkr_blob.data(), glen};
        for (int k = 0; k < 2; k++) { const uint64_t m = r.u64(); r.skip(m * 16 + 24); }
        const uint64_t nr = r.u64();
        for (uint64_t k = 0; k < nr; k++) {
            r.skip(64);
            const uint64_t np = r.u64();
            for (uint64_t q = 0; q < np; q++) { const uint64_t nc = r.u64(); r.skip(nc * 16); }
            r.skip(16);
            const uint64_t pl = r.u64();
            r.skip(pl * 16 + 16);
        }
        SP1HIP_REQUIRE(r.u64() == (uint64_t)L, "internal: GKR point dimension");
        for (auto& z : zeta) z = r.ext();
        SP1HIP_REQUIRE(r.u64() == (uint64_t)n_chips, "internal: GKR chip count");
        for (int c = 0; c < n_chips; c++) {
            r.skip(r.u64());
            const uint64_t mw = r.u64();
            for (uint64_t k = 0; k < mw; k++) openings.push_back(r.ext());
            r.skip(16);
            if (r.p[r.o++]) {
                const uint64_t pw = r.u64();
                for (uint64_t k = 0; k < pw; k++) openings.push_back(r.ext());
                r.skip(16);
            }
        }
    }
    sh_t[2] = std::chrono::steady_clock::now();
    marks.next("zerocheck");
    const kb::Ext batching = challenger_sample_ext(ch), gkr_batch = challenger_sample_ext(ch);
    sp1hip_ext_t c_batching, c_gkr;
    memcpy(&c_batching, &batching, 16);
    memcpy(&c_gkr, &gkr_batch, 16);
    std::vector<uint8_t> zc_blob(zc_size);
    size_t zlen = zc_size;
    SP1HIP_TRY(sp1hip_zerocheck_prove(zc.data(), n_chips, L, reinterpret_cast<const sp1hip_ext_t*>(zeta.data()),
                                      reinterpret_cast<const sp1hip_ext_t*>(openings.data()), c_batching, c_gkr, h_publics, n_publics, ch,
                                      zc_blob.data(), &zlen, stream));
    std::vector<kb::Ext> z_row(L), prep_claims, main_claims;
    std::vector<std::vector<kb::Ext>> chip_evals(n_chips);
    {
        Reader r{zc_blob.data(), zlen};
        const uint64_t np = r.u64();
        for (uint64_t q = 0; q < np; q++) { const uint64_t nc = r.u64(); r.skip(nc * 16); }
        r.skip(16);
        SP1HIP_REQUIRE(r.u64() == (uint64_t)L, "internal: zerocheck point dimension");
        for (auto& z : z_row) z = r.ext();
        r.skip(16);
        SP1HIP_REQUIRE(r.o == zc_sumcheck_size, "internal: zerocheck sumcheck size");
        SP1HIP_REQUIRE(r.u64() == (uint64_t)n_chips, "internal: zerocheck chip count");
        for (int c = 0; c < n_chips; c++) {
            const uint64_t w = r.u64();
            SP1HIP_REQUIRE(w == (uint64_t)chips[c].main_width + chips[c].prep_width, "internal: zerocheck opening width");
            for (uint64_t k = 0; k < w; k++) chip_evals[c].push_back(r.ext());
            prep_claims.insert(prep_claims.end(), chip_evals[c].begin(), chip_evals[c].begin() + chips[c].prep_width);
            main_claims.insert(main_claims.end(), chip_evals[c].begin() + chips[c].prep_width, chip_evals[c].end());
        }
    }
    sh_t[3] = std::chrono::steady_clock::now();
    marks.next("evaluation_proof");
    std::vector<kb::Ext> claims = prep_claims;
    claims.insert(claims.end(), main_claims.begin(), main_claims.end());
    const size_t per_round[2] = {prep_claims.size(), main_claims.size()};
    sp1hip_stacked_data_t* rounds[2] = {preprocessed, main_data};
    SP1HIP_REQUIRE(need >= jag_size, "internal error: shard proof sizes");
    uint8_t* const jag_at = h_proof + (need - jag_size);
    size_t jlen = jag_size;
    SP1HIP_TRY(sp1hip_jagged_prove(reinterpret_cast<const sp1hip_ext_t*>(z_row.data()), L, rounds, 2,
                                   reinterpret_cast<const sp1hip_ext_t*>(claims.data()), per_round, params.fri, ch, jag_at, &jlen,
                                   stream));
    SP1HIP_REQUIRE(jlen == jag_size, "internal error: jagged proof size");
    (void)s;

    sh_t[4] = std::chrono::steady_clock::now();
    marks.next("proof_bytes");
    std::vector<uint8_t> out;
    out.reserve(need - jag_size);
    put_u64(out, n_publics);
    for (int i = 0; i < n_publics; i++) put_felt(out, h_publics[i]);
    for (int k = 0; k < 8; k++) put_felt(out, main_commit[k]);
    out.insert(out.end(), gkr_blob.begin(), gkr_blob.begin() + glen);
    out.insert(out.end(), zc_blob.begin(), zc_blob.begin() + zc_sumcheck_size);
    put_u64(out, n_chips);
    for (int c = 0; c < n_chips; c++) {
        const size_t nl = strlen(chips[c].name);
        put_u64(out, nl);
        out.insert(out.end(), chips[c].name, chips[c].name + nl);
        put_u64(out, chips[c].prep_width);
        for (uint32_t k = 0; k < chips[c].prep_width; k++) for (int q = 0; q < 4; q++) put_felt(out, chip_evals[c][k].c[q]);
        put_u64(out, chips[c].main_width);
        for (uint32_t k = 0; k < chips[c].main_width; k++) for (int q = 0; q < 4; q++) put_felt(out, chip_evals[c][chips[c].prep_width + k].c[q]);
        put_u64(out, L + 1);
        for (int b = L; b >= 0; b--) put_felt(out, ((chips[c].real_rows >> b) & 1) ? kb::R1 : 0u);
    }
    if (out.size() + jlen != need) {
        set_error("internal error: shard proof size %zu != expected %zu", out.size() + jlen, need);
        return SP1HIP_ERROR_RUNTIME;
    }
    memcpy(h_proof, out.data(), out.size());
    *proof_len = need;
    challenger_restore(challenger, ch);
    if (sh_timing) {
        sh_t[5] = std::chrono::steady_clock::now();
        const auto ms = [&](int a, int b) { return std::chrono::duration<double, std::milli>(sh_t[b] - sh_t[a]).count(); };
        uint64_t miss_n1 = 0, miss_b1 = 0;
        arena_miss_stats(&miss_n1, &miss_b1);
        fprintf(stderr, "[sp1hip shard] prologue %.3f ms | commit %.3f | LogUp-GKR %.3f | zerocheck %.3f | evaluation proof %.3f | proof bytes %.3f | %llu arena misses (%.1f MB)\n",
                std::chrono::duration<double, std::milli>(sh_t[0] - sh_entry).count(), ms(0, 1), ms(1, 2), ms(2, 3), ms(3, 4), ms(4, 5),
                (unsigned long long)(miss_n1 - miss_n0), (double)(miss_b1 - miss_b0) / 1e6);
    }
    wait_plan.ok = true;
    return SP1HIP_SUCCESS;
}


struct sp1hip_pk_s {
    sp1hip_stacked_data_t* preprocessed = nullptr;
    sp1hip_vk_t vk{};
    sp1hip_shard_params_t params{};
    ~sp1hip_pk_s() { if (preprocessed) sp1hip_stacked_data_free(preprocessed); }
};

int sp1hip_setup(const sp1hip_table_t* preprocessed_tables, int n_tables, const uint32_t pc_start[3],
                 const uint32_t initial_global_cumulative_sum[14], uint32_t enable_untrusted_programs,
                 sp1hip_shard_params_t params, sp1hip_pk_t** out, sp1hip_stream_t stream) {
    SP1HIP_REQUIRE(preprocessed_tables && n_tables > 0 && pc_start && initial_global_cumulative_sum && out, "null argument");
    for (int i = 0; i < 3; i++) SP1HIP_REQUIRE(pc_start[i] < kb::P, "pc_start not reduced");
    for (int i = 0; i < 14; i++) SP1HIP_REQUIRE(initial_global_cumulative_sum[i] < kb::P, "cumulative sum not reduced");
    SP1HIP_REQUIRE(enable_untrusted_programs < kb::P, "flag not reduced");
    std::unique_ptr<sp1hip_pk_s> pk(new sp1hip_pk_s());
    SP1HIP_TRY(sp1hip_jagged_commit(preprocessed_tables, n_tables, params.max_log_row_count, params.log_stacking_height,
                                    params.batch_size, params.fri.log_blowup, pk->vk.preprocessed_commit, &pk->preprocessed, stream));
    memcpy(pk->vk.pc_start, pc_start, 12);
    memcpy(pk->vk.initial_global_cumulative_sum, initial_global_cumulative_sum, 56);
    pk->vk.enable_untrusted_programs = enable_untrusted_programs;
    pk->params = params;
    *out = pk.release();
    return SP1HIP_SUCCESS;
}

void sp1hip_pk_free(sp1hip_pk_t* pk) { delete pk; }

int sp1hip_pk_vk(const sp1hip_pk_t* pk, sp1hip_vk_t* out) {
    SP1HIP_REQUIRE(pk && out, "null argument");
    *out = pk->vk;
    return SP1HIP_SUCCESS;
}

int sp1hip_vk_observe_into(const sp1hip_vk_t* vk, sp1hip_challenger_t* challenger) {
    SP1HIP_REQUIRE(vk && challenger, "null argument");
    for (int k = 0; k < 8; k++) challenger_observe(challenger, vk->preprocessed_commit[k]);
    for (int k = 0; k < 3; k++) challenger_observe(challenger, vk->pc_start[k]);
    for (int k = 0; k < 14; k++) challenger_observe(challenger, vk->initial_global_cumulative_sum[k]);
    challenger_observe(challenger, vk->enable_untrusted_programs);
    for (int k = 0; k < 6; k++) challenger_observe(challenger, 0u);
    return SP1HIP_SUCCESS;
}

int sp1hip_prove_shard_with_pk(const sp1hip_pk_t* pk, const sp1hip_shard_chip_t* chips, int n_chips, const uint32_t* h_publics,
                               int n_publics, const uint32_t* pow_witnesses, int n_pow_witnesses, uint8_t* h_proof, size_t* proof_len,
                               sp1hip_stream_t stream) {
    SP1HIP_REQUIRE(pk && proof_len, "null argument");
    sp1hip_challenger_t* ch = nullptr;
    SP1HIP_TRY(sp1hip_challenger_new(&ch));
    struct ChGuard { sp1hip_challenger_t* c; ~ChGuard() { sp1hip_challenger_free(c); } } guard{ch};
    SP1HIP_TRY(sp1hip_vk_observe_into(&pk->vk, ch));
    if (n_pow_witnesses) SP1HIP_TRY(sp1hip_challenger_inject_pow_witnesses(ch, pow_witnesses, n_pow_witnesses));
    return sp1hip_prove_shard(chips, n_chips, h_publics, n_publics, pk->preprocessed, pk->params, ch, h_proof, proof_len, stream);
}

}
```

### sp1_amd/csrc/zerocheck.hip

```cpp
#include <algorithm>
#include <array>
#include <cstring>
#include <functional>
#include <memory>
#include <mutex>
#include <unordered_map>
#include <vector>

#include "device_ctx.hpp"
#include "round_sync.hpp"
#include "zc_device.hpp"
#include "zc_poseidon2.hpp"
#include "zc_keccak.hpp"
#include "zc_mul.hpp"
#include "zc_poly.hpp"

namespace sp1hip {

template <bool FIRST, int MAXR> struct RegFile;

typedef uint32_t zc_lds_word_t __attribute__((address_space(3)));
typedef uint32_t zc_lds_quad_t __attribute__((ext_vector_type(4), address_space(3)));
typedef uint32_t zc_quad_t __attribute__((ext_vector_type(4)));
template <> struct RegFile<true, 0> {
    zc_lds_word_t* base;
    uint32_t stride;
    __device__ __forceinline__ uint32_t get(uint32_t i) const { return base[i * stride]; }
    __device__ __forceinline__ void set(uint32_t i, uint32_t v) { base[i * stride] = v; }
};
template <> struct RegFile<false, 0> {
    zc_lds_quad_t* base;
    uint32_t stride;
    __device__ __forceinline__ kb::Ext get(uint32_t i) const { const zc_quad_t v = base[i * stride]; return kb::Ext{{v.x, v.y, v.z, v.w}}; }
    __device__ __forceinline__ void set(uint32_t i, const kb::Ext& v) { zc_quad_t q = {v.c[0], v.c[1], v.c[2], v.c[3]}; base[i * stride] = q; }
};

constexpr uint32_t ZC_GKR_FLAG = 0x100u;
constexpr uint32_t ZC_A_PREV = 0x1000u, ZC_B_PREV = 0x2000u;
constexpr uint32_t ZC_DST_TEMP = 0x4000u;
constexpr uint32_t ZC_TOUCH = 9;
constexpr uint32_t ZC_ADDC = 10, ZC_SUBC = 11, ZC_CSUB = 12, ZC_MULC = 13;
constexpr uint32_t ZC_MADC = 14;
constexpr uint32_t ZC_RSUB = 15;
constexpr uint32_t ZC_MAD = 16, ZC_MSB = 17;
constexpr uint32_t ZC_MONO_MIN_TERMS = 1024;
constexpr uint32_t ZC_CHUNK_LIMIT = 96;
constexpr uint32_t ZC_CHUNK_HARD_MAX = 320;
constexpr uint32_t ZC_FINE_LIMIT = 32, ZC_FINE_MAX_TERMS = 64;
constexpr uint32_t ZC_FORK_MAX_BLOCKS = 1u << 30;
constexpr uint32_t ZC_MAX_PAIRS = 131072;
constexpr uint32_t ZC_SMALL_ROUND_WGS = 16384;

typedef uint32_t zc_word_t __attribute__((ext_vector_type(4)));
typedef const zc_word_t __attribute__((address_space(4)))* zc_const_prog_t;

constexpr int ZC_BIV_NODES = 12;
struct ZcBivNode { uint32_t cx, cy, cxy; };
__host__ __device__ __forceinline__ ZcBivNode zc_biv_node(uint32_t e) {
    constexpr uint32_t XS[12] = {0, 0, 1, 1, 2, 2, 2, 2, 4, 4, 4, 4}, YS[12] = {2, 4, 2, 4, 0, 1, 2, 4, 0, 1, 2, 4};
    return ZcBivNode{XS[e], YS[e], XS[e] * YS[e]};
}
__host__ __device__ __forceinline__ uint32_t zc_reduce36(uint64_t v) {
    const uint32_t t = (uint32_t)(v >> 31), lo = (uint32_t)v & 0x7fffffffu;
    const uint32_t r = lo + t * 0xffffffu;
    return kb::umin(r, r - kb::P);
}
__host__ __device__ __forceinline__ uint32_t zc_biv_interp(uint32_t r00, uint32_t r01, uint32_t r10, uint32_t r11, const ZcBivNode& nd) {
    const uint32_t dy = kb::sub(r01, r00), dx = kb::sub(r10, r00), dxy = kb::sub(kb::sub(r11, r10), dy);
    return zc_reduce36((uint64_t)r00 + (uint64_t)nd.cx * dx + (uint64_t)nd.cy * dy + (uint64_t)nd.cxy * dxy);
}
__device__ __forceinline__ uint32_t zc_biv_leaf(const uint32_t* tbl, uint32_t col, uint32_t rows, uint32_t q, const ZcBivNode& nd) {
    const zc_global_words_t g = (zc_global_words_t)tbl + (size_t)col * rows;
    const uint32_t r = 4 * q;
    const uint32_t r00 = g[r], r01 = r + 1 < rows ? g[r + 1] : 0u, r10 = r + 2 < rows ? g[r + 2] : 0u, r11 = r + 3 < rows ? g[r + 3] : 0u;
    return zc_biv_interp(r00, r01, r10, r11, nd);
}

struct KT4 {
    using T = kb::Ext;
    static __device__ __forceinline__ T zero() { return kb::ext_zero(); }
    static __device__ __forceinline__ T from_f(uint32_t x) { return kb::Ext{{x, x, x, x}}; }
    static __device__ __forceinline__ T add(const T& a, const T& b) { return kb::ext_add(a, b); }
    static __device__ __forceinline__ T sub(const T& a, const T& b) { return kb::ext_sub(a, b); }
    static __device__ __forceinline__ T mul(const T& a, const T& b) {
        return kb::Ext{{kb::mul(a.c[0], b.c[0]), kb::mul(a.c[1], b.c[1]), kb::mul(a.c[2], b.c[2]), kb::mul(a.c[3], b.c[3])}};
    }
};
struct KC4 {
    static __device__ __forceinline__ kb::Ext addc(const kb::Ext& a, uint32_t c) { return kb::Ext{{kb::add(a.c[0], c), kb::add(a.c[1], c), kb::add(a.c[2], c), kb::add(a.c[3], c)}}; }
    static __device__ __forceinline__ kb::Ext subc(const kb::Ext& a, uint32_t c) { return kb::Ext{{kb::sub(a.c[0], c), kb::sub(a.c[1], c), kb::sub(a.c[2], c), kb::sub(a.c[3], c)}}; }
    static __device__ __forceinline__ kb::Ext csub(uint32_t c, const kb::Ext& a) { return kb::Ext{{kb::sub(c, a.c[0]), kb::sub(c, a.c[1]), kb::sub(c, a.c[2]), kb::sub(c, a.c[3])}}; }
    static __device__ __forceinline__ kb::Ext mulc(const kb::Ext& a, uint32_t c) { return kb::ext_mul_base(a, c); }
};
// ... 1741 lines not shown
            size_t mono_instr = 0;
            for (auto& ck : np->mono) mono_instr += ck.prog.size() / 4;
            fprintf(stderr, "[sp1hip zc] chip %d: %u ssa instrs, %u+%u cols -> undivided program %zu words, %u registers\n",
                    chip_index, n_instr, main_width, prep_width, mono_instr, best_regs);
        }
        SP1HIP_TRY(allocate_registers(sched.data(), n_sched, &np->prog, &np->n_regs));
        std::vector<uint32_t> sched_f = sched;
        drop_hinted(sched_f);
        SP1HIP_TRY(build_chunks(sched_f.data(), n_sched, main_width, prep_width, ZC_CHUNK_LIMIT, &np->chunks, ZC_CHUNK_HARD_MAX, &np->macros, &np->polys));
        SP1HIP_TRY(build_chunks(sched_f.data(), n_sched, main_width, prep_width, ZC_FINE_LIMIT, &np->fine, ZC_FINE_LIMIT, &np->macros, &np->polys));
        np->sched = sched;
        if (!np->macros.empty()) {
            std::vector<uint32_t> row(main_width), prow(std::max<uint32_t>(prep_width, 1u)), want(asserts_total(program, n_instr), 0u);
            uint64_t x = 0x9E3779B97F4A7C15ull ^ h;
            auto rnd = [&]() { x ^= x << 13; x ^= x >> 7; x ^= x << 17; return (uint32_t)(x % kb::P); };
            for (auto& v : row) v = rnd();
            for (auto& v : prow) v = rnd();
            uint32_t n_pub = 1;
            for (uint32_t k = 0; k < n_instr; k++) if (program[3 * k] == ZC_PUBLIC) n_pub = std::max(n_pub, program[3 * k + 1] + 1);
            std::vector<uint32_t> pub(n_pub, 0u);
            eval_words_row(np->prog.data(), np->prog.size() / 4, np->n_regs, row.data(), prow.data(), pub.data(),
                           [&](uint32_t idx, uint32_t v) { if (idx < want.size()) want[idx] = v; });
            for (const ZcMacro& m : np->macros) {
                bool ok = true;
                uint32_t n_seen = 0;
                macro_eval_row(m, np->polys, row.data(), [&](uint32_t j, uint32_t v) {
                    n_seen++;
                    const bool same = m.first_constraint + j < want.size() && want[m.first_constraint + j] == v;
                    if (!same && zc_debug)
                        fprintf(stderr, "[sp1hip zc] hint kind %u: constraint %u + %u: pieces give %08x, the program %08x\n", m.kind, m.first_constraint, j,
                                v, m.first_constraint + j < want.size() ? want[m.first_constraint + j] : 0u);
                    ok &= same;
                });
                SP1HIP_REQUIRE(ok && n_seen == m.n_constraints(), "a fused-kernel hint does not match the constraints it annotates");
            }
        }
        plan = np;
        std::lock_guard<std::mutex> lk(plan_mutex);
        if (plan_cache.size() > 4096) plan_cache.clear();
        plan_cache[h] = plan;
    }
    *out = plan;
    return SP1HIP_SUCCESS;
}

template <bool FIRST> static inline size_t zc_rf_lane_bytes(uint32_t n_regs) { return (size_t)n_regs * (FIRST ? 4 : 16); }
constexpr size_t ZC_LDS_CU = 160 * 1024;
constexpr size_t ZC_LDS_BUDGET = ZC_LDS_CU;

template <bool FIRST> static inline uint32_t zc_wg_for(uint32_t n_regs, size_t other_lds) {
    uint32_t best = 0, best_lanes = 0;
    for (uint32_t wg = 256; wg >= 64; wg >>= 1) {
        const size_t per_wg = other_lds + zc_rf_lane_bytes<FIRST>(n_regs) * wg;
        if (per_wg > ZC_LDS_CU) continue;
        const uint32_t lanes = (uint32_t)std::min<size_t>(ZC_LDS_CU / per_wg, 2048 / wg) * wg;
        if (lanes > best_lanes) { best_lanes = lanes; best = wg; }
    }
    return best;
}

template <bool FIRST>
static int launch_round(uint32_t max_regs, bool staged, const ZcDesc* d_descs, int n_descs, uint32_t block_lo, uint32_t n_blocks,
                        uint32_t max_instr, const uint32_t* eq, uint32_t eq_len, const uint32_t* publics, uint32_t* partial, hipStream_t s) {
    const size_t lds = 32 * 4 + (staged ? (size_t)max_instr * 16 : 0);
    const dim3 grid(n_blocks * 3);
    const uint32_t wg = zc_wg_for<FIRST>(max_regs, lds);
    SP1HIP_REQUIRE(wg != 0, "internal: a register file that does not fit LDS reached the launch (plan_round cuts such programs finer)");
    const size_t total = lds + zc_rf_lane_bytes<FIRST>(max_regs) * wg;
    if (staged) {
        auto kern = zc_round_kernel<FIRST, 0, true>;
        if (total > 48 * 1024) SP1HIP_TRY(ensure_dynamic_lds((const void*)kern, (int)ZC_LDS_BUDGET));
        hipLaunchKernelGGL(kern, grid, dim3(wg), total, s, d_descs, n_descs, eq, eq_len, publics, partial, (uint32_t)(lds / 4), block_lo);
    } else {
        auto kern = zc_round_kernel<FIRST, 0, false>;
        if (total > 48 * 1024) SP1HIP_TRY(ensure_dynamic_lds((const void*)kern, (int)ZC_LDS_BUDGET));
        hipLaunchKernelGGL(kern, grid, dim3(wg), total, s, d_descs, n_descs, eq, eq_len, publics, partial, (uint32_t)(lds / 4), block_lo);
    }
    SP1HIP_LAUNCH_CHECK();
    return SP1HIP_SUCCESS;
}

struct ByteOut {
    std::vector<uint8_t> b;
    void u64(uint64_t v) { for (int i = 0; i < 8; i++) b.push_back((uint8_t)(v >> (8 * i))); }
    void ext(const Ext& e) {
        for (int k = 0; k < 4; k++) { uint32_t c = kb::from_monty(e.c[k]); for (int i = 0; i < 4; i++) b.push_back((uint8_t)(c >> (8 * i))); }
    }
};

}

using namespace sp1hip;

struct sp1hip_challenger_s;
namespace sp1hip {
void challenger_observe(sp1hip_challenger_t* ch, uint32_t x);
kb::Ext challenger_sample_ext(sp1hip_challenger_t* ch);
void challenger_restore(sp1hip_challenger_t* dst, const sp1hip_challenger_t* src);
static int launch_biv_round(uint32_t max_regs, bool staged, const ZcDesc* d_descs, int n_descs, uint32_t block_lo, uint32_t n_blocks,
                            uint32_t max_instr, const uint32_t* eq, uint32_t eq_len, const uint32_t* publics, uint32_t* partial, hipStream_t s) {
    const size_t lds = 32 * 4 + (staged ? (size_t)max_instr * 16 : 0);
    const dim3 grid(n_blocks * ZC_BIV_GROUPS);
    const uint32_t wg = zc_wg_for<false>(max_regs, lds);
    SP1HIP_REQUIRE(wg != 0, "internal: a register file that does not fit LDS reached the launch (plan_round cuts such programs finer)");
    const size_t total = lds + zc_rf_lane_bytes<false>(max_regs) * wg;
    if (staged) {
        auto kern = zc_biv_round_kernel<0, true>;
        if (total > 48 * 1024) SP1HIP_TRY(ensure_dynamic_lds((const void*)kern, (int)ZC_LDS_BUDGET));
        hipLaunchKernelGGL(kern, grid, dim3(wg), total, s, d_descs, n_descs, eq, eq_len, publics, partial, (uint32_t)(lds / 4), block_lo);
    } else {
        auto kern = zc_biv_round_kernel<0, false>;
        if (total > 48 * 1024) SP1HIP_TRY(ensure_dynamic_lds((const void*)kern, (int)ZC_LDS_BUDGET));
        hipLaunchKernelGGL(kern, grid, dim3(wg), total, s, d_descs, n_descs, eq, eq_len, publics, partial, (uint32_t)(lds / 4), block_lo);
    }
    SP1HIP_LAUNCH_CHECK();
    return SP1HIP_SUCCESS;
}

int eq_prefix_tables_soa_async(const kb::Ext* h_point, int d, uint32_t* d_out, hipStream_t s);
}

constexpr int ZC_N_FORK = 2;

static int zerocheck_prove_impl(const sp1hip_zc_chip_t* chips, int n_chips, int max_log_row_count,
                               const sp1hip_ext_t* h_zeta, const sp1hip_ext_t* h_openings, sp1hip_ext_t alpha_c,
                               sp1hip_ext_t gkr_c, const uint32_t* h_publics, int n_publics,
                               sp1hip_challenger_t* challenger, uint8_t* h_proof, size_t* proof_len,
                               sp1hip_stream_t stream) {
    SP1HIP_REQUIRE(chips && n_chips > 0 && h_zeta && h_openings && challenger && proof_len, "null argument");
    SP1HIP_REQUIRE(max_log_row_count >= 1 && max_log_row_count <= 30, "max_log_row_count out of range");
    SP1HIP_REQUIRE(h_publics || n_publics == 0, "null publics");
    ActiveProver active;
    const int L = max_log_row_count;
    size_t total_w = 0;
    for (int i = 0; i < n_chips; i++) {
        SP1HIP_REQUIRE(chips[i].program || chips[i].n_instr == 0, "null constraint program");
        SP1HIP_REQUIRE(chips[i].real_rows <= ((uint64_t)1 << L), "chip taller than 2^max_log_row_count");
        SP1HIP_REQUIRE(chips[i].real_rows == 0 || (chips[i].d_main || chips[i].main_width == 0), "null main trace");
        SP1HIP_REQUIRE(chips[i].real_rows == 0 || (chips[i].d_prep || chips[i].prep_width == 0), "null preprocessed trace");
        total_w += chips[i].main_width + chips[i].prep_width;
    }
    const size_t need = 8 + (size_t)L * (8 + 80) + 16 + 8 + (size_t)L * 16 + 16 + 8 + (size_t)n_chips * 8 + total_w * 16;
    if (!h_proof || *proof_len < need) {
        *proof_len = need;
        set_error("sp1hip_zerocheck_prove: proof buffer too small, need %zu bytes", need);
        return SP1HIP_ERROR_BUFFER_TOO_SMALL;
    }
    hipStream_t s = S(stream);
    const DeviceCtx* ctx;
    SP1HIP_TRY(get_device_ctx(&ctx));
    const bool zc_timing = env_flag("SP1HIP_ZC_TIMING", false);
    const auto zc_t0 = std::chrono::steady_clock::now();
    auto zc_t1 = zc_t0, zc_t2 = zc_t0;
    const Ext alpha{{alpha_c.c[0], alpha_c.c[1], alpha_c.c[2], alpha_c.c[3]}};
    const Ext gkr{{gkr_c.c[0], gkr_c.c[1], gkr_c.c[2], gkr_c.c[3]}};
    std::vector<uint32_t> publics(h_publics, h_publics + n_publics);
    DevBuf d_publics;
    SP1HIP_TRY(d_publics.alloc((size_t)n_publics * 4, s));

    int max_constraints = 0;
    for (int i = 0; i < n_chips; i++) max_constraints = std::max<int>(max_constraints, chips[i].num_constraints);
    std::vector<Ext> pows(max_constraints);
    { Ext cur = kb::ext_one(); for (auto& x : pows) { x = cur; cur = cur * alpha; } }

    Mailbox mb;
    SP1HIP_TRY(mb.init(s));
    RoundSyncHost rsync;
    SP1HIP_TRY(rsync.init(s));
    PinnedStage stage;
    SP1HIP_TRY(stage.init(s));
    if (n_publics) SP1HIP_TRY(stage.upload(d_publics.p, publics.data(), (size_t)n_publics * 4));
    std::vector<uint32_t> blob;
    Ext rho = kb::ext_zero();
    bool have_rho = false;
    std::vector<kb::Ext> poly_scratch[2];
    std::vector<std::unique_ptr<ChipState>> st;
    std::vector<Ext> claims;
    size_t oo = 0;
    for (int i = 0; i < n_chips; i++) {
        std::unique_ptr<ChipState> c(new ChipState());
        c->in = &chips[i];
        uint32_t asserts = 0;
        for (uint32_t k = 0; k < chips[i].n_instr; k++) {
            const uint32_t op = chips[i].program[3 * k], a = chips[i].program[3 * k + 1];
            SP1HIP_REQUIRE(op <= ZC_ASSERT_ZERO || op == ZC_HINT, "bad opcode in constraint program");
            if (op == ZC_ASSERT_ZERO) asserts++;
            if (op == ZC_LOAD_MAIN) SP1HIP_REQUIRE(a < chips[i].main_width, "main column out of range");
            if (op == ZC_LOAD_PREP) SP1HIP_REQUIRE(a < chips[i].prep_width, "preprocessed column out of range");
            if (op == ZC_PUBLIC) SP1HIP_REQUIRE((int)a < n_publics, "public value index out of range");
        }
        SP1HIP_REQUIRE(asserts == chips[i].num_constraints, "num_constraints does not match the program");
        {
            std::shared_ptr<const ZcPlan> plan;
            SP1HIP_TRY(zc_get_plan(chips[i].program, chips[i].n_instr, chips[i].main_width, chips[i].prep_width, i, &plan, chips[i].real_rows));
            c->prog = plan->prog; c->n_regs = plan->n_regs; c->chunks = plan->chunks; c->mono = plan->mono; c->fine = plan->fine;
            c->macros = plan->macros;
            c->plan = plan;
        }
        c->alpha_pows.assign(pows.begin(), pows.begin() + chips[i].num_constraints);
        std::reverse(c->alpha_pows.begin(), c->alpha_pows.end());
        { Ext cur = gkr; for (uint32_t k = 0; k < chips[i].main_width + chips[i].prep_width; k++) { c->gkr_pows.push_back(cur); cur = cur * gkr; } }
        c->pad_adj = eval_zero_row(*c, publics.data());
        Ext claim = kb::ext_zero();
        for (uint32_t k = 0; k < chips[i].main_width + chips[i].prep_width; k++, oo++) {
            const Ext o{{h_openings[oo].c[0], h_openings[oo].c[1], h_openings[oo].c[2], h_openings[oo].c[3]}};
            claim = claim + o * c->gkr_pows[k];
        }
        claims.push_back(claim);
        c->rows = chips[i].real_rows;
        c->num_vars = (uint32_t)L;
        c->eq_adj = kb::ext_one();
        c->vgeq = VGeq{(uint32_t)chips[i].real_rows, kb::ext_one(), kb::ext_zero()};
        c->d_main = chips[i].d_main;
        c->d_prep = chips[i].d_prep;
        auto pad4 = [&]() { while (blob.size() & 3) blob.push_back(0); };
        pad4();
        c->off_prog = blob.size();
        for (auto& ck : c->chunks) {
            c->chunk_off.push_back((uint32_t)((blob.size() - c->off_prog) / 4));
            blob.insert(blob.end(), ck.prog.begin(), ck.prog.end());
        }
        for (auto& ck : c->mono) {
            c->mono_off.push_back((uint32_t)((blob.size() - c->off_prog) / 4));
            blob.insert(blob.end(), ck.prog.begin(), ck.prog.end());
        }
        for (auto& ck : c->fine) {
            c->fine_off.push_back((uint32_t)((blob.size() - c->off_prog) / 4));
            blob.insert(blob.end(), ck.prog.begin(), ck.prog.end());
        }
        pad4();
        c->off_alpha = blob.size();
        for (const Ext& e : c->alpha_pows) blob.insert(blob.end(), e.c, e.c + 4);
        c->off_gkr = blob.size();
        for (const Ext& e : c->gkr_pows) blob.insert(blob.end(), e.c, e.c + 4);
        c->poly_off.assign(c->macros.size(), 0);
        for (size_t mi = 0; mi < c->macros.size(); mi++) {
            const ZcMacro& m = c->macros[mi];
            if (m.kind != ZC_HINT_POLY) continue;
            if (!have_rho) {
                SP1HIP_REQUIRE(!kb::ext_eq(alpha, kb::ext_zero()), "the batching challenge is zero");
                rho = kb::ext_inv(alpha); have_rho = true;
            }
            while (blob.size() & 7) blob.push_back(0);
            c->poly_off[mi] = blob.size();
            zc_poly_table(c->plan->polys[m.aux0], c->plan->poly_segs[m.aux0], c->alpha_pows.data() + m.first_constraint, rho, &blob, poly_scratch);
        }
        st.push_back(std::move(c));
    }
    DevBuf d_blob;
    SP1HIP_TRY(d_blob.alloc(std::max<size_t>(blob.size(), 4) * 4, s));
    SP1HIP_TRY(stage.upload(d_blob.p, blob.data(), blob.size() * 4));
    for (auto& c : st) {
        c->p_prog = d_blob.u32() + c->off_prog;
        c->p_alpha = d_blob.u32() + c->off_alpha;
        c->p_gkr = d_blob.u32() + c->off_gkr;
        c->p_blob = d_blob.u32();
    }

    std::vector<Ext> zeta(L);
    memcpy(zeta.data(), h_zeta, (size_t)L * 16);
    const Ext lambda = challenger_sample_ext(challenger);
    DevBuf d_eq_all;
    SP1HIP_TRY(d_eq_all.alloc(((size_t)1 << L) * 16, s));
    SP1HIP_TRY(eq_prefix_tables_soa_async(zeta.data(), L - 1, d_eq_all.u32(), s));
    std::vector<UniPoly> msgs;
    std::vector<Ext> point;
    std::vector<Ext> round_claims = claims;
    std::vector<std::array<uint32_t, 16>> sums(n_chips);
    std::vector<uint32_t> h_sums((size_t)n_chips * 64);
    DevBuf d_partial, d_sums;
    size_t partial_cap = 0;
    SP1HIP_TRY(d_sums.alloc((size_t)n_chips * 256, s));
    DevBuf d_fold[2];
    {
        size_t words[2] = {4, 4};
        for (int half = 0; half < 2; half++)
            for (int i = 0; i < n_chips; i++) {
                uint64_t rows = chips[i].real_rows;
                for (int k = 0; k < half && rows; k++) rows = (rows + 1) / 2;
                if (rows == 0) continue;
                const uint64_t out_rows = (rows + 1) / 2;
                for (uint32_t width : {chips[i].main_width, chips[i].prep_width})
                    if (width) words[half] += (((size_t)out_rows * width * 4 + 3) & ~(size_t)3);
            }
        SP1HIP_TRY(d_fold[0].alloc(words[0] * 4, s));
        SP1HIP_TRY(d_fold[1].alloc(words[1] * 4, s));
    }
    zc_t1 = std::chrono::steady_clock::now();
    auto zc_iter_t = zc_t1;
    double zc_plan_ms = 0, zc_wait_ms = 0, zc_uni_ms = 0;
    static const struct CubicBasis {
        uint32_t c[4][4];
        CubicBasis() {
            const int num[4][4] = {{-8, 14, -7, 1}, {0, 8, -6, 1}, {0, 4, -5, 1}, {0, 2, -3, 1}};
            const int den[4] = {-8, 3, -4, 24};
            for (int k = 0; k < 4; k++) {
                const uint32_t dm = kb::to_monty(den[k] < 0 ? kb::P - (uint32_t)(-den[k]) : (uint32_t)den[k]);
                const uint32_t dinv = kb::ext_inv(kb::ext_from_base(dm)).c[0];
                for (int d = 0; d < 4; d++) {
                    const uint32_t nm = kb::to_monty(num[k][d] < 0 ? kb::P - (uint32_t)(-num[k][d]) : (uint32_t)num[k][d]);
                    c[k][d] = kb::mul(nm, dinv);
                }
            }
        }
    } cubic;
    std::vector<Ext> lam_pows(n_chips);
    { Ext cur = kb::ext_one(); for (int i = n_chips - 1; i >= 0; i--) { lam_pows[i] = cur; cur = cur * lambda; } }
    std::vector<std::array<Ext, 4>> ys(n_chips);
    Ext claim_w[4];
    Ext pending_a = kb::ext_zero(), pending_last = kb::ext_zero();
    bool claims_pending = false;
    auto update_claims = [&]() {
        if (!claims_pending) return;
        claims_pending = false;
        for (int i = 0; i < n_chips; i++) {
            ChipState& c = *st[i];
            c.vgeq = c.vgeq.fix(pending_a);
            if (c.rows == 0) { round_claims[i] = kb::ext_zero(); continue; }
            round_claims[i] = ys[i][0] * claim_w[0] + ys[i][1] * claim_w[1] + ys[i][2] * claim_w[2] + ys[i][3] * claim_w[3];
            c.eq_adj = c.eq_adj * (pending_a * pending_last + (kb::ext_one() - pending_a) * (kb::ext_one() - pending_last));
        }
    };
    auto round_messages = [&](const Ext& last, const std::vector<std::array<Ext, 3>>& hv) -> Ext {
        update_claims();
        const Ext b_node = (kb::ext_one() - last) * kb::ext_inv(kb::ext_one() - (last + last));
        Ext inv_xb[4];
        {
            const Ext dx[4] = {kb::ext_zero() - b_node, kb::ext_one() - b_node, ext_c(2) - b_node, ext_c(4) - b_node};
            const Ext p01 = dx[0] * dx[1], p012 = p01 * dx[2], p0123 = p012 * dx[3];
            Ext run = kb::ext_inv(p0123);
            inv_xb[3] = run * p012; run = run * dx[3];
            inv_xb[2] = run * p01; run = run * dx[2];
            inv_xb[1] = run * dx[0];
            inv_xb[0] = run * dx[1];
        }
        const Ext three = ext_c(3), seven = ext_c(7);
        const Ext f0 = kb::ext_one() - last, f2 = last * three - kb::ext_one(), f4 = last * seven - three;
        Ext Y[4] = {kb::ext_zero(), kb::ext_zero(), kb::ext_zero(), kb::ext_zero()};
        for (int i = 0; i < n_chips; i++) {
            if (st[i]->rows == 0) continue;
            const Ext y0 = hv[i][0] * f0;
            ys[i] = {y0, round_claims[i] - y0, hv[i][1] * f2, hv[i][2] * f4};
            for (int k = 0; k < 4; k++) Y[k] = Y[k] + ys[i][k] * lam_pows[i];
        }
        UniPoly rlc(n_chips ? 5 : 1, kb::ext_zero());
        if (n_chips) {
            const Ext z[4] = {Y[0] * inv_xb[0], Y[1] * inv_xb[1], Y[2] * inv_xb[2], Y[3] * inv_xb[3]};
            Ext g[4];
            for (int d = 0; d < 4; d++) {
                Ext acc = kb::ext_mul_base(z[0], cubic.c[0][d]);
                for (int k = 1; k < 4; k++) acc = acc + kb::ext_mul_base(z[k], cubic.c[k][d]);
                g[d] = acc;
            }
            rlc[0] = kb::ext_zero() - b_node * g[0];
            for (int d = 1; d < 4; d++) rlc[d] = g[d - 1] - b_node * g[d];
            rlc[4] = g[3];
        }
        for (auto& cf : rlc)
            for (int k = 0; k < 4; k++) challenger_observe(challenger, cf.c[k]);
        msgs.push_back(rlc);
        const Ext a_r = challenger_sample_ext(challenger);
        point.insert(point.begin(), a_r);
        {
            const Ext a2 = a_r * a_r, a3 = a2 * a_r, ab = a_r - b_node;
            for (int k = 0; k < 4; k++) {
                const Ext ck = kb::ext_from_base(cubic.c[k][0]) + kb::ext_mul_base(a_r, cubic.c[k][1]) + kb::ext_mul_base(a2, cubic.c[k][2]) + kb::ext_mul_base(a3, cubic.c[k][3]);
                claim_w[k] = ab * ck * inv_xb[k];
            }
        }
        pending_a = a_r; pending_last = last; claims_pending = true;
// ... 499 lines not shown
                    SP1HIP_LAUNCH_CHECK();
                }
                if (ln.kind == (int)ZC_HINT_KECCAK) {
                    if (r == 0) hipLaunchKernelGGL((zc_macro_kernel<true, 5u>), dim3(macro_n[5] * 3), dim3(256), 0, ls, dd, n_descs, d_eq.u32(), eq_len, d_partial.u32(), macro_lo[5], dctx->d_rc);
                    else hipLaunchKernelGGL((zc_macro_kernel<false, 5u>), dim3(macro_n[5] * 3), dim3(256), 0, ls, dd, n_descs, d_eq.u32(), eq_len, d_partial.u32(), macro_lo[5], dctx->d_rc);
                    SP1HIP_LAUNCH_CHECK();
                }
#undef SP1HIP_ZC_MACRO_LAUNCH
                if (ln.kind == (int)ZC_MACRO_BOTH_SEPTIC) {
                    hipLaunchKernelGGL((zc_macro_kernel<false, ZC_MACRO_BOTH_SEPTIC>), dim3((macro_n[2] + macro_n[3]) * 3), dim3(256), 0, ls, dd, n_descs, d_eq.u32(), eq_len, d_partial.u32(), macro_lo[2], dctx->d_rc);
                    SP1HIP_LAUNCH_CHECK();
                }
            }
            if (forked)
                for (int k = 0; k < N_FORK; k++)
                    if (fork_used[k]) {
                        SP1HIP_HIP(hipEventRecord(fork_ev[1 + k], fork_s[k]));
                        SP1HIP_HIP(hipStreamWaitEvent(s, fork_ev[1 + k], 0));
                    }
            if (direct) { rsync.pending = true; mb.pending = true; }
            if (r == 0) hipLaunchKernelGGL(zc_reduce_kernel<true>, dim3(n_ranges), dim3(256), 0, s, d_ranges_p, d_partial.u32(), d_eq.u32(), eq_len, d_sums.u32(), rs_pub, mb.seq + 1);
            else hipLaunchKernelGGL(zc_reduce_kernel<false>, dim3(n_ranges), dim3(256), 0, s, d_ranges_p, d_partial.u32(), d_eq.u32(), eq_len, d_sums.u32(), rs_pub, mb.seq + 1);
            SP1HIP_LAUNCH_CHECK();
            if (r + 1 < L && (int)plans.size() == r + 1) {
                plans.emplace_back(new RoundPlan());
                SP1HIP_TRY(plan_round(r + 1, rp.rows_next, rp.main_next, rp.prep_next, *plans.back(), false));
                SP1HIP_TRY(upload_plan(*plans.back(), (r + 1) & 1));
            }
            const auto zc_w0 = std::chrono::steady_clock::now();
            if (zc_timing) zc_plan_ms += std::chrono::duration<double, std::milli>(zc_w0 - zc_iter_t).count();
            if (direct) { SP1HIP_TRY(mb.wait_next(h_sums.data(), (size_t)n_ranges * 16)); rsync.pending = false; }
            else SP1HIP_TRY(mb.fetch(d_sums.p, (size_t)n_ranges * 16, h_sums.data()));
            if (zc_timing) { zc_iter_t = std::chrono::steady_clock::now(); zc_wait_ms += std::chrono::duration<double, std::milli>(zc_iter_t - zc_w0).count(); }
        }
        if (r + 1 < L && (int)plans.size() == r + 1) {
            plans.emplace_back(new RoundPlan());
            SP1HIP_TRY(plan_round(r + 1, rp.rows_next, rp.main_next, rp.prep_next, *plans.back(), false));
            SP1HIP_TRY(upload_plan(*plans.back(), (r + 1) & 1));
        }
        {
            std::vector<char> have(n_chips, 0);
            for (size_t k = 0; k < desc_chip.size(); k++) {
                const int ci = desc_chip[k];
                const uint32_t* src = h_sums.data() + k * 16;
                if (!have[ci]) { memcpy(sums[ci].data(), src, 64); have[ci] = 1; }
                else for (int w = 0; w < 12; w++) sums[ci][w] = kb::add(sums[ci][w], src[w]);
            }
        }
        std::vector<std::array<Ext, 3>> hv(n_chips);
        {
            const Ext two = ext_c(2), four = ext_c(4);
            for (int i = 0; i < n_chips; i++) {
                ChipState& c = *st[i];
                if (c.rows == 0) continue;
                const size_t th = (size_t)((c.rows + 1) / 2) - 1;
                const Ext eq_th{{sums[i][12], sums[i][13], sums[i][14], sums[i][15]}};
                const Ext msb = c.eq_adj * eq_th;
                const Ext y0s{{sums[i][0], sums[i][1], sums[i][2], sums[i][3]}}, y2s{{sums[i][4], sums[i][5], sums[i][6], sums[i][7]}},
                    y4s{{sums[i][8], sums[i][9], sums[i][10], sums[i][11]}};
                const Ext v0 = c.vgeq.fix(kb::ext_zero()).at(th), v2 = c.vgeq.fix(two).at(th), v4 = c.vgeq.fix(four).at(th);
                const Ext pm = c.pad_adj * msb;
                hv[i] = {y0s * c.eq_adj - pm * v0, y2s * c.eq_adj - pm * v2, y4s * c.eq_adj - pm * v4};
            }
        }
        const Ext a_r = round_messages(last, hv);
        if (zc_timing) { const auto now = std::chrono::steady_clock::now(); zc_uni_ms += std::chrono::duration<double, std::milli>(now - zc_iter_t).count(); zc_iter_t = now; }
        if (!fds.empty()) {
            ScopedTimer tm("zerocheck_fix", s);
            if (r == 0) hipLaunchKernelGGL(zc_fix_kernel<true>, dim3(fix_blocks), dim3(256), 0, s, d_fix_p, (int)fds.size(), a_r);
            else hipLaunchKernelGGL(zc_fix_kernel<false>, dim3(fix_blocks), dim3(256), 0, s, d_fix_p, (int)fds.size(), a_r);
            SP1HIP_LAUNCH_CHECK();
            for (size_t k = 0; k < fds.size(); k++) {
                ChipState& c = *st[owner[k].first];
                if (owner[k].second) c.d_main = fresh[k]; else c.d_prep = fresh[k];
            }
        }
        update_claims();
        for (int i = 0; i < n_chips; i++)
            if (st[i]->rows) st[i]->rows = (st[i]->rows + 1) / 2;
    }
    update_claims();
    zc_t2 = std::chrono::steady_clock::now();
    ByteOut w;
    w.u64((uint64_t)L);
    for (auto& m : msgs) { w.u64(m.size()); for (auto& cf : m) w.ext(cf); }
    Ext claimed = kb::ext_zero(), final_eval = kb::ext_zero();
    for (auto& cl : claims) claimed = claimed * lambda + cl;
    for (int i = 0; i < n_chips; i++) final_eval = final_eval * lambda + round_claims[i];
    w.ext(claimed);
    w.u64(point.size());
    for (auto& x : point) w.ext(x);
    w.ext(final_eval);
    w.u64((uint64_t)n_chips);
    std::vector<std::vector<Ext>> chip_evals(n_chips);
    {
        std::vector<ZcGatherDesc> gd;
        size_t total_words = 0;
        for (int i = 0; i < n_chips; i++) {
            ChipState& c = *st[i];
            const uint32_t wp = c.in->prep_width, wm = c.in->main_width;
            if (c.rows && wp) gd.push_back({c.d_prep, wp * 4, (uint32_t)total_words});
            total_words += (size_t)wp * 4;
            if (c.rows && wm) gd.push_back({c.d_main, wm * 4, (uint32_t)total_words});
            total_words += (size_t)wm * 4;
        }
        std::vector<uint32_t> flat(total_words, 0);
        if (!gd.empty()) {
            DevBuf d_gd, d_flat;
            SP1HIP_TRY(d_gd.alloc(gd.size() * sizeof(ZcGatherDesc), s));
            SP1HIP_TRY(d_flat.alloc(total_words * 4, s));
            SP1HIP_HIP(hipMemsetAsync(d_flat.p, 0, total_words * 4, s));
            SP1HIP_TRY(stage.upload(d_gd.p, gd.data(), gd.size() * sizeof(ZcGatherDesc)));
            hipLaunchKernelGGL(zc_gather_kernel, dim3((unsigned)gd.size()), dim3(256), 0, s, (const ZcGatherDesc*)d_gd.p, d_flat.u32());
            SP1HIP_LAUNCH_CHECK();
            SP1HIP_TRY(mb.fetch(d_flat.p, total_words, flat.data()));
        }
        size_t off = 0;
        for (int i = 0; i < n_chips; i++) {
            const uint32_t wtot = st[i]->in->prep_width + st[i]->in->main_width;
            for (uint32_t k = 0; k < wtot; k++, off += 4)
                chip_evals[i].push_back(Ext{{flat[off], flat[off + 1], flat[off + 2], flat[off + 3]}});
            w.u64(chip_evals[i].size());
            for (auto& e : chip_evals[i]) w.ext(e);
        }
    }
    challenger_observe(challenger, kb::to_monty((uint32_t)n_chips));
    for (int i = 0; i < n_chips; i++) {
        const uint32_t wp = st[i]->in->prep_width, wm = st[i]->in->main_width;
        challenger_observe(challenger, kb::to_monty(wp));
        for (uint32_t k = 0; k < wp; k++) for (int q = 0; q < 4; q++) challenger_observe(challenger, chip_evals[i][k].c[q]);
        challenger_observe(challenger, kb::to_monty(wm));
        for (uint32_t k = 0; k < wm; k++) for (int q = 0; q < 4; q++) challenger_observe(challenger, chip_evals[i][wp + k].c[q]);
    }
    if (w.b.size() != need) { set_error("internal error: zerocheck proof size %zu != %zu", w.b.size(), need); return SP1HIP_ERROR_RUNTIME; }
    memcpy(h_proof, w.b.data(), need);
    *proof_len = need;
    if (zc_timing) {
        const auto ms = [](std::chrono::steady_clock::time_point a, std::chrono::steady_clock::time_point b) { return std::chrono::duration<double, std::milli>(b - a).count(); };
        fprintf(stderr, "[sp1hip zerocheck] set-up %.3f ms | %d rounds %.3f ms (planning + launches %.3f, waiting for the sums %.3f, univariates + transcript %.3f) | openings + proof %.3f ms\n",
                ms(zc_t0, zc_t1), L, ms(zc_t1, zc_t2), zc_plan_ms, zc_wait_ms, zc_uni_ms, ms(zc_t2, std::chrono::steady_clock::now()));
    }
    return SP1HIP_SUCCESS;
}

namespace sp1hip {
template <bool FIRST>
__global__ __launch_bounds__(256) void fix_last_variable_kernel(const uint32_t* __restrict__ in, uint32_t rows, uint32_t width,
                                                                kb::Ext alpha, const uint32_t* __restrict__ padding,
                                                                uint32_t* __restrict__ out) {
    using K = KT<FIRST>;
    const uint32_t out_rows = (rows + 1) / 2;
    const size_t t = (size_t)blockIdx.x * 256u + threadIdx.x;
    if (t >= (size_t)out_rows * width) return;
    const uint32_t c = (uint32_t)(t / out_rows), i = (uint32_t)(t % out_rows);
    typename K::T x = K::load(in, c, rows, 2 * i), y;
    if (2 * i + 1 < rows) y = K::load(in, c, rows, 2 * i + 1);
    else if (!padding) y = K::zero();
    else y = K::load(padding, c, 1, 0);
    const kb::Ext r = kb::ext_add(K::scale(alpha, K::sub(y, x)), K::to_ext(x));
#pragma unroll
    for (int q = 0; q < 4; q++) out[((size_t)c * 4 + q) * out_rows + i] = r.c[q];
}
}

extern "C" int sp1hip_zerocheck_biv_interp_host(uint32_t r00, uint32_t r01, uint32_t r10, uint32_t r11, uint32_t node, uint32_t* out) {
    SP1HIP_REQUIRE(out && node < (uint32_t)ZC_BIV_NODES, "node out of range");
    SP1HIP_REQUIRE(r00 < kb::P && r01 < kb::P && r10 < kb::P && r11 < kb::P, "word not reduced");
    *out = zc_biv_interp(r00, r01, r10, r11, zc_biv_node(node));
    return SP1HIP_SUCCESS;
}

extern "C" int sp1hip_zerocheck_plan_eval(const uint32_t* program, uint32_t n_instr, uint32_t main_width, uint32_t prep_width,
                                          const uint32_t* main_row, const uint32_t* prep_row, const uint32_t* publics,
                                          uint32_t n_publics, int form, uint32_t* out_values, uint32_t n_constraints,
                                          uint32_t* out_stats) {
    SP1HIP_REQUIRE(program || n_instr == 0, "null program");
    SP1HIP_REQUIRE(out_values || n_constraints == 0, "null output");
    SP1HIP_REQUIRE(form >= 0 && form <= 3, "form: 0 whole program, 1 chunks, 2 undivided, 3 fine");
    uint32_t asserts = 0;
    for (uint32_t k = 0; k < n_instr; k++) {
        const uint32_t op = program[3 * k], a = program[3 * k + 1];
        SP1HIP_REQUIRE(op <= ZC_ASSERT_ZERO || op == ZC_HINT, "bad opcode in constraint program");
        if (op == ZC_ASSERT_ZERO) asserts++;
        if (op == ZC_LOAD_MAIN) SP1HIP_REQUIRE(a < main_width && main_row, "main column out of range");
        if (op == ZC_LOAD_PREP) SP1HIP_REQUIRE(a < prep_width && prep_row, "preprocessed column out of range");
        if (op == ZC_PUBLIC) SP1HIP_REQUIRE(a < n_publics && publics, "public value index out of range");
    }
    SP1HIP_REQUIRE(asserts == n_constraints, "n_constraints does not match the program");
    std::shared_ptr<const ZcPlan> plan;
    SP1HIP_TRY(zc_get_plan(program, n_instr, main_width, prep_width, -1, &plan));
    std::vector<uint32_t> seen(n_constraints, 0);
    auto on_assert = [&](uint32_t idx, uint32_t v) { if (idx < n_constraints) { out_values[idx] = v; seen[idx]++; } };
    uint32_t words = 0, pieces = 0, regs = 0;
    if (form == 0) {
        eval_words_row(plan->prog.data(), plan->prog.size() / 4, plan->n_regs, main_row, prep_row, publics, on_assert);
        words = (uint32_t)(plan->prog.size() / 4); pieces = 1; regs = plan->n_regs;
    } else {
        const std::vector<Chunk>& cks = form == 1 ? plan->chunks : form == 2 ? plan->mono : plan->fine;
        for (const Chunk& ck : cks) {
            eval_words_row(ck.prog.data(), ck.prog.size() / 4, ck.n_regs, main_row, prep_row, publics, on_assert);
            words += (uint32_t)(ck.prog.size() / 4); pieces++; regs = std::max(regs, ck.n_regs);
        }
    }
    if (form != 0) {
        for (const ZcMacro& m : plan->macros) {
            macro_eval_row(m, plan->polys, main_row, [&](uint32_t j, uint32_t v) { on_assert(m.first_constraint + j, v); });
            pieces += m.n_pieces();
        }
    }
    for (uint32_t k = 0; k < n_constraints; k++) SP1HIP_REQUIRE(seen[k] == 1, "a constraint was not evaluated exactly once");
    if (out_stats) { out_stats[0] = words; out_stats[1] = pieces; out_stats[2] = regs; }
    return SP1HIP_SUCCESS;
}

extern "C" int sp1hip_zerocheck_poly_check(const uint32_t* program, uint32_t n_instr, uint32_t main_width, uint32_t prep_width,
                                           const uint32_t* main_row, sp1hip_ext_t alpha_c, sp1hip_ext_t* out_collapsed,
                                           sp1hip_ext_t* out_direct, uint32_t* n_identities) {
    SP1HIP_REQUIRE(program && main_row && out_collapsed && out_direct && n_identities, "null argument");
    for (uint32_t k = 0; k < n_instr; k++) SP1HIP_REQUIRE(program[3 * k] <= ZC_ASSERT_ZERO || program[3 * k] == ZC_HINT, "bad opcode in constraint program");
    std::shared_ptr<const ZcPlan> plan;
    SP1HIP_TRY(zc_get_plan(program, n_instr, main_width, prep_width, -1, &plan));
    const Ext alpha{{alpha_c.c[0], alpha_c.c[1], alpha_c.c[2], alpha_c.c[3]}};
    SP1HIP_REQUIRE(!kb::ext_eq(alpha, kb::ext_zero()), "the batching challenge is zero");
    const uint32_t n_c = asserts_total(program, n_instr);
    std::vector<Ext> pows(n_c);
    { Ext cur = kb::ext_one(); for (uint32_t k = n_c; k-- > 0;) { pows[k] = cur; cur = cur * alpha; } }
    const Ext rho = kb::ext_inv(alpha);
    Ext collapsed = kb::ext_zero(), direct = kb::ext_zero();
    std::vector<kb::Ext> scratch[2];
    uint32_t count = 0;
    for (const ZcMacro& m : plan->macros) {
        if (m.kind != ZC_HINT_POLY) continue;
        count++;
        const ZcPoly& pl = plan->polys[m.aux0];
        std::vector<uint32_t> tb;
        zc_poly_table(pl, plan->poly_segs[m.aux0], pows.data() + m.first_constraint, rho, &tb, scratch);
        size_t off = ZC_POLY_HDR;
        auto form = [&](uint32_t n, bool with_const) -> Ext {
            Ext f = kb::ext_zero();
            if (with_const) { f = Ext{{tb[off + 4], tb[off + 5], tb[off + 6], tb[off + 7]}}; off += ZC_POLY_ENTRY; }
            for (uint32_t k = 0; k < n; k++, off += ZC_POLY_ENTRY) f = f + kb::ext_mul_base(Ext{{tb[off + 4], tb[off + 5], tb[off + 6], tb[off + 7]}}, main_row[tb[off]]);
            return f;
        };
        Ext v = kb::ext_zero();
        for (uint32_t t = 0; t < tb[0]; t++) {
            Ext p = form(tb[4 + 3 * t], true) * form(tb[5 + 3 * t], true);
            if (tb[6 + 3 * t] != ZC_POLY_NONE) p = p * form(tb[6 + 3 * t], true);
            v = v + p;
        }
        v = v + form(tb[1], true) + form(tb[2], false);
        collapsed = collapsed + v;
        zc_poly_eval_row(pl, main_row, [&](uint32_t k, uint32_t c) { direct = direct + kb::ext_mul_base(pows[m.first_constraint + k], c); });
    }
    memcpy(out_collapsed->c, collapsed.c, 16);
    memcpy(out_direct->c, direct.c, 16);
    *n_identities = count;
    return SP1HIP_SUCCESS;
}

extern "C" int sp1hip_fix_last_variable(const uint32_t* d_in, uint64_t rows, uint32_t width, int in_is_ext, sp1hip_ext_t alpha,
                                        const uint32_t* d_padding, uint32_t* d_out, sp1hip_stream_t stream) {
    SP1HIP_REQUIRE(rows < ((uint64_t)1 << 32), "too many rows");
    if (rows == 0 || width == 0) return SP1HIP_SUCCESS;
    SP1HIP_REQUIRE(d_in && d_out && d_in != d_out, "bad buffers");
    const kb::Ext a{{alpha.c[0], alpha.c[1], alpha.c[2], alpha.c[3]}};
    const uint64_t total = ((rows + 1) / 2) * width;
    SP1HIP_REQUIRE((total + 255) / 256 < ((uint64_t)1 << 31), "table too large for one launch");
    const dim3 grid((unsigned)((total + 255) / 256));
    if (in_is_ext) hipLaunchKernelGGL(fix_last_variable_kernel<false>, grid, dim3(256), 0, S(stream), d_in, (uint32_t)rows, width, a, d_padding, d_out);
    else hipLaunchKernelGGL(fix_last_variable_kernel<true>, grid, dim3(256), 0, S(stream), d_in, (uint32_t)rows, width, a, d_padding, d_out);
    SP1HIP_LAUNCH_CHECK();
    return SP1HIP_SUCCESS;
}

extern "C" int sp1hip_zerocheck_prove(const sp1hip_zc_chip_t* chips, int n_chips, int max_log_row_count,
                                      const sp1hip_ext_t* h_zeta, const sp1hip_ext_t* h_openings, sp1hip_ext_t alpha,
                                      sp1hip_ext_t gkr_batch, const uint32_t* h_publics, int n_publics,
                                      sp1hip_challenger_t* challenger, uint8_t* h_proof, size_t* proof_len,
                                      sp1hip_stream_t stream) {
    sp1hip_challenger_t* backup = nullptr;
    if (challenger) SP1HIP_TRY(sp1hip_challenger_clone(challenger, &backup));
    const int st = zerocheck_prove_impl(chips, n_chips, max_log_row_count, h_zeta, h_openings, alpha, gkr_batch, h_publics,
                                        n_publics, challenger, h_proof, proof_len, stream);
    if (st != SP1HIP_SUCCESS && challenger) challenger_restore(challenger, backup);
    sp1hip_challenger_free(backup);
    return st;
}
```

Baseline: 97.55 million.

## Cache parsed interaction programs and hand stage results over without re-parsing proof bytes

```diff
diff --git a/sp1_amd/csrc/gkr.hip b/sp1_amd/csrc/gkr.hip
--- a/sp1_amd/csrc/gkr.hip
+++ b/sp1_amd/csrc/gkr.hip
@@ -3,7 +3,9 @@
 #include <chrono>
 #include <cstring>
 #include <memory>
+#include <mutex>
 #include <string>
+#include <unordered_map>
 #include <vector>
 
 #include "device_ctx.hpp"
@@ -15,6 +17,7 @@
 void gkr_host_round_fold(const uint32_t* tab, uint32_t* out, size_t stride, size_t real_pairs, const uint32_t alpha[4]);
 }
 #include "round_sync.hpp"
+#include "stage_handover.hpp"
 #include "tensor_table.hpp"
 
 namespace sp1hip {
@@ -623,9 +626,10 @@
 
 struct Bytes {
     std::vector<uint8_t> b;
-    void u64(uint64_t v) { for (int i = 0; i < 8; i++) b.push_back((uint8_t)(v >> (8 * i))); }
-    void felt(uint32_t m) { const uint32_t v = kb::from_monty(m); for (int i = 0; i < 4; i++) b.push_back((uint8_t)(v >> (8 * i))); }
-    void ext(const Ext& e) { for (int k = 0; k < 4; k++) felt(e.c[k]); }
+    void raw(const void* src, size_t k) { const uint8_t* p = (const uint8_t*)src; b.insert(b.end(), p, p + k); }
+    void u64(uint64_t v) { raw(&v, 8); }
+    void felt(uint32_t m) { const uint32_t v = kb::from_monty(m); raw(&v, 4); }
+    void ext(const Ext& e) { uint32_t v[4]; for (int k = 0; k < 4; k++) v[k] = kb::from_monty(e.c[k]); raw(v, 16); }
 };
 
 void observe_ext(sp1hip_challenger_t* ch, const Ext& e) { for (int k = 0; k < 4; k++) challenger_observe(ch, e.c[k]); }
@@ -642,6 +646,116 @@
     const uint32_t* d_prep;
 };
 
+struct IntHead {
+    uint32_t kind;
+    std::vector<std::pair<uint32_t, uint32_t>> consts;
+};
+struct ParsedMachine {
+    std::vector<uint32_t> key;
+    std::vector<uint32_t> chip_k, chip_int0;
+    std::vector<uint32_t> int_chip;
+    size_t max_arity = 0;
+    std::vector<uint32_t> flat;
+    std::vector<size_t> poff;
+    std::vector<IntHead> heads;
+};
+
+void machine_key(const sp1hip_gkr_chip_t* chips, int n_chips, std::vector<uint32_t>* key) {
+    size_t n = 0;
+    for (int c = 0; c < n_chips; c++) n += 3 + (chips[c].interactions ? chips[c].n_words : 0);
+    key->clear();
+    key->reserve(n);
+    for (int c = 0; c < n_chips; c++) {
+        key->insert(key->end(), {chips[c].n_words, chips[c].main_width, chips[c].prep_width});
+        if (chips[c].interactions) key->insert(key->end(), chips[c].interactions, chips[c].interactions + chips[c].n_words);
+    }
+}
+
+uint64_t hash_words(const std::vector<uint32_t>& w) {
+    uint64_t h[4] = {0xcbf29ce484222325ull, 0x84222325cbf29ce4ull, 0x9ce484222325cbf2ull, 0x2325cbf29ce48422ull};
+    size_t i = 0;
+    for (; i + 4 <= w.size(); i += 4)
+        for (int k = 0; k < 4; k++) h[k] = (h[k] ^ w[i + k]) * 0x100000001b3ull;
+    for (; i < w.size(); i++) h[0] = (h[0] ^ w[i]) * 0x100000001b3ull;
+    uint64_t r = w.size();
+    for (int k = 0; k < 4; k++) r = (r ^ h[k]) * 0x100000001b3ull;
+    return r;
+}
+
+int parse_machine(const sp1hip_gkr_chip_t* chips, int n_chips, ParsedMachine* out) {
+    for (int c = 0; c < n_chips; c++) {
+        const sp1hip_gkr_chip_t& ci = chips[c];
+        SP1HIP_REQUIRE(ci.n_words >= 1, "empty interaction program");
+        const uint32_t* p = ci.interactions;
+        const uint32_t* end = p + ci.n_words;
+        const uint32_t ni = *p++;
+        out->chip_int0.push_back((uint32_t)out->poff.size());
+        out->chip_k.push_back(ni);
+        auto vcol = [&](std::vector<uint32_t>& dst) -> bool {
+            if (p + 2 > end) return false;
+            const uint32_t nt = p[0];
+            if (p[1] >= kb::P || p + 2 + 3 * (size_t)nt > end) return false;
+            dst.push_back(nt);
+            dst.push_back(kb::to_monty(p[1]));
+            p += 2;
+            for (uint32_t t = 0; t < nt; t++, p += 3) {
+                if (p[0] > 1 || p[2] >= kb::P) return false;
+                if (p[1] >= (p[0] ? ci.main_width : ci.prep_width)) return false;
+                dst.push_back(p[0]); dst.push_back(p[1]); dst.push_back(kb::to_monty(p[2]));
+            }
+            return true;
+        };
+        std::vector<uint32_t> body, val;
+        for (uint32_t i = 0; i < ni; i++) {
+            SP1HIP_REQUIRE(p + 3 <= end, "truncated interaction program");
+            const uint32_t is_send = p[0], kind = p[1], nv = p[2];
+            SP1HIP_REQUIRE(is_send <= 1 && kind < kb::P && nv < 4096, "bad interaction header");
+            p += 3;
+            body.clear();
+            SP1HIP_REQUIRE(vcol(body), "bad multiplicity column");
+            IntHead head{kb::to_monty(kind), {}};
+            uint32_t live = 0;
+            for (uint32_t j = 0; j < nv; j++) {
+                val.clear();
+                SP1HIP_REQUIRE(vcol(val), "bad value column (index or weight out of range)");
+                if (val[0] == 0) { head.consts.emplace_back(1 + j, val[1]); continue; }
+                live++;
+                body.push_back(1 + j);
+                body.insert(body.end(), val.begin(), val.end());
+            }
+            out->max_arity = std::max<size_t>(out->max_arity, nv + 1);
+            out->poff.push_back(out->flat.size());
+            out->flat.insert(out->flat.end(), {is_send, live, 0u, 0u, 0u, 0u});
+            out->flat.insert(out->flat.end(), body.begin(), body.end());
+            out->heads.push_back(std::move(head));
+            out->int_chip.push_back((uint32_t)c);
+        }
+        SP1HIP_REQUIRE(p == end, "trailing words in interaction program");
+    }
+    return SP1HIP_SUCCESS;
+}
+
+int parsed_machine_for(const sp1hip_gkr_chip_t* chips, int n_chips, std::shared_ptr<const ParsedMachine>* out) {
+    static std::mutex mutex;
+    static std::unordered_map<uint64_t, std::shared_ptr<const ParsedMachine>> cache;
+    std::vector<uint32_t> key;
+    machine_key(chips, n_chips, &key);
+    const uint64_t h = hash_words(key);
+    {
+        std::lock_guard<std::mutex> lk(mutex);
+        auto it = cache.find(h);
+        if (it != cache.end() && it->second->key == key) { *out = it->second; return SP1HIP_SUCCESS; }
+    }
+    std::shared_ptr<ParsedMachine> pm(new ParsedMachine());
+    SP1HIP_TRY(parse_machine(chips, n_chips, pm.get()));
+    pm->key = std::move(key);
+    std::lock_guard<std::mutex> lk(mutex);
+    if (cache.size() >= 256) cache.clear();
+    cache[h] = pm;
+    *out = pm;
+    return SP1HIP_SUCCESS;
+}
+
 constexpr uint32_t MAX_TILES = 512;
 uint32_t tiles_for(uint64_t threads) { return (uint32_t)std::min<uint64_t>(std::max<uint64_t>((threads + 255) / 256, 1), MAX_TILES); }
 }
@@ -650,10 +764,8 @@
 using namespace sp1hip;
 using namespace sp1hip::gkr;
 
-extern "C" {
-
-int sp1hip_logup_gkr_prove(const sp1hip_gkr_chip_t* chips, int n_chips, int max_log_row_count, sp1hip_challenger_t* challenger,
-                           uint8_t* h_proof, size_t* proof_len, sp1hip_stream_t stream) {
+static int logup_gkr_prove_impl(const sp1hip_gkr_chip_t* chips, int n_chips, int max_log_row_count, sp1hip_challenger_t* challenger,
+                                uint8_t* h_proof, size_t* proof_len, sp1hip_stream_t stream, GkrHandover* handover) {
     SP1HIP_REQUIRE(chips && n_chips > 0 && challenger && proof_len, "bad argument");
     const int L = max_log_row_count;
     SP1HIP_REQUIRE(L >= 1 && L <= 30, "max_log_row_count out of range");
@@ -668,9 +780,7 @@
     };
 
     std::vector<ChipInfo> info(n_chips);
-    struct ParsedInt { uint32_t is_send, kind; std::vector<uint32_t> mult; std::vector<std::vector<uint32_t>> values; };
-    std::vector<ParsedInt> progs;
-    size_t max_arity = 0, total_cols = 0;
+    size_t total_cols = 0;
     for (int c = 0; c < n_chips; c++) {
         const sp1hip_gkr_chip_t& ci = chips[c];
         SP1HIP_REQUIRE(ci.name && ci.interactions, "null chip field");
@@ -678,41 +788,16 @@
         SP1HIP_REQUIRE(ci.real_rows == 0 || ci.main_width == 0 || ci.d_main, "null main trace");
         SP1HIP_REQUIRE(ci.real_rows == 0 || ci.prep_width == 0 || ci.d_prep, "null preprocessed trace");
         if (c) SP1HIP_REQUIRE(strcmp(chips[c - 1].name, ci.name) < 0, "chips must be sorted by name (BTreeSet order)");
-        info[c] = ChipInfo{ci.name, (uint32_t)ci.real_rows, 0, ci.main_width, ci.prep_width, (uint32_t)progs.size(), ci.d_main, ci.d_prep};
-        const uint32_t* p = ci.interactions;
-        const uint32_t* end = p + ci.n_words;
-        SP1HIP_REQUIRE(ci.n_words >= 1, "empty interaction program");
-        const uint32_t ni = *p++;
-        info[c].k = ni;
-        auto vcol = [&](std::vector<uint32_t>& out) -> bool {
-            if (p + 2 > end) return false;
-            const uint32_t nt = p[0];
-            if (p[1] >= kb::P || p + 2 + 3 * (size_t)nt > end) return false;
-            out.push_back(nt);
-            out.push_back(kb::to_monty(p[1]));
-            p += 2;
-            for (uint32_t t = 0; t < nt; t++, p += 3) {
-                if (p[0] > 1 || p[2] >= kb::P) return false;
-                if (p[1] >= (p[0] ? ci.main_width : ci.prep_width)) return false;
-                out.push_back(p[0]); out.push_back(p[1]); out.push_back(kb::to_monty(p[2]));
-            }
-            return true;
-        };
-        for (uint32_t i = 0; i < ni; i++) {
-            SP1HIP_REQUIRE(p + 3 <= end, "truncated interaction program");
-            const uint32_t nv = p[2];
-            SP1HIP_REQUIRE(p[0] <= 1 && p[1] < kb::P && nv < 4096, "bad interaction header");
-            ParsedInt pi{p[0], p[1], {}, std::vector<std::vector<uint32_t>>(nv)};
-            p += 3;
-            SP1HIP_REQUIRE(vcol(pi.mult), "bad multiplicity column");
-            for (uint32_t j = 0; j < nv; j++) SP1HIP_REQUIRE(vcol(pi.values[j]), "bad value column (index or weight out of range)");
-            max_arity = std::max<size_t>(max_arity, nv + 1);
-            progs.push_back(std::move(pi));
-        }
-        SP1HIP_REQUIRE(p == end, "trailing words in interaction program");
         total_cols += (size_t)ci.main_width + ci.prep_width;
     }
-    const uint32_t K = (uint32_t)progs.size();
+    std::shared_ptr<const ParsedMachine> machine;
+    SP1HIP_TRY(parsed_machine_for(chips, n_chips, &machine));
+    for (int c = 0; c < n_chips; c++)
+        info[c] = ChipInfo{chips[c].name, (uint32_t)chips[c].real_rows, machine->chip_k[c], chips[c].main_width, chips[c].prep_width,
+                           machine->chip_int0[c], chips[c].d_main, chips[c].d_prep};
+    const size_t max_arity = machine->max_arity;
+    mark("interaction programs parsed");
+    const uint32_t K = (uint32_t)machine->poff.size();
     SP1HIP_REQUIRE(K >= 1, "no interactions in the shard");
     const int niv = log2_ceil(K), beta_seed_dim = log2_ceil(max_arity);
     const uint32_t W = 1u << niv;
@@ -738,16 +823,18 @@
     struct ChGuard { sp1hip_challenger_t* c; ~ChGuard() { sp1hip_challenger_free(c); } } guard{ch};
 
     uint32_t witness = 0;
+    mark("size + challenger clone");
     SP1HIP_TRY(sp1hip_challenger_grind(ch, 12, &witness, stream));
+    mark("grind hand-over");
     const Ext alpha = challenger_sample_ext(ch);
     std::vector<Ext> beta_seed(beta_seed_dim);
     for (auto& b : beta_seed) b = challenger_sample_ext(ch);
     (void)challenger_sample_ext(ch);
     const std::vector<Ext> betas = partial_lagrange_host(beta_seed);
+    mark("challenges sampled");
 
     auto rows_at = [&](uint32_t h, int l) -> uint32_t { return (uint32_t)(((uint64_t)h + (((uint64_t)1 << (L - l)) - 1)) >> (L - l)); };
-    std::vector<uint32_t> int_chip(K);
-    for (int c = 0; c < n_chips; c++) for (uint32_t i = 0; i < info[c].k; i++) int_chip[info[c].int0 + i] = c;
+    const std::vector<uint32_t>& int_chip = machine->int_chip;
     std::vector<size_t> level_entries(L + 2, 0);
     for (int l = 1; l <= L; l++) for (uint32_t i = 0; i < K; i++) level_entries[l] += rows_at(info[int_chip[i]].rows, l);
     std::vector<DeviceBuf> lvN(L + 1), lvD(L + 1);
@@ -760,7 +847,7 @@
     auto n_ptr = [&](int l, uint32_t i) -> void* { return (char*)lvN[l].p + off[l][i] * (l == L ? 4 : 16); };
     auto d_ptr = [&](int l, uint32_t i) -> Ext* { return lvD[l].ext() + off[l][i]; };
 
-    mark("parse + level buffers");
+    mark("level buffers");
     const uint32_t FLAT_MAX_SLOTS = (uint32_t)env_uint("SP1HIP_GKR_FLAT_SLOTS", 65536);
     size_t n_passes_total = 0;
     for (int v = 1; v <= L - 1; v++) n_passes_total += (size_t)(v + 1) / 2 + 1;
@@ -774,29 +861,20 @@
     SP1HIP_TRY(side_stage.init(side));
     PinnedStage stage;
     SP1HIP_TRY(stage.init(s));
+    mark("side stream + staging");
     DeviceBuf d_progs, d_betas, d_descs;
     uint32_t max_rows = 0;
     bool fused_tree = false;
     std::vector<uint32_t> flat;
     std::vector<IntDesc> descs(K);
     {
-        std::vector<size_t> poff(K);
+        const std::vector<size_t>& poff = machine->poff;
+        flat = machine->flat;
         for (uint32_t i = 0; i < K; i++) {
-            poff[i] = flat.size();
-            const ParsedInt& pi = progs[i];
-            Ext head = alpha + kb::ext_mul_base(betas[0], kb::to_monty(pi.kind));
-            uint32_t live = 0;
-            for (size_t j = 0; j < pi.values.size(); j++) {
-                if (pi.values[j][0] == 0) head = head + kb::ext_mul_base(betas[1 + j], pi.values[j][1]);
-                else live++;
-            }
-            flat.insert(flat.end(), {pi.is_send, live, head.c[0], head.c[1], head.c[2], head.c[3]});
-            flat.insert(flat.end(), pi.mult.begin(), pi.mult.end());
-            for (size_t j = 0; j < pi.values.size(); j++) {
-                if (pi.values[j][0] == 0) continue;
-                flat.push_back((uint32_t)(1 + j));
-                flat.insert(flat.end(), pi.values[j].begin(), pi.values[j].end());
-            }
+            const IntHead& ih = machine->heads[i];
+            Ext head = alpha + kb::ext_mul_base(betas[0], ih.kind);
+            for (auto& jc : ih.consts) head = head + kb::ext_mul_base(betas[jc.first], jc.second);
+            memcpy(&flat[poff[i] + 2], head.c, 16);
         }
         SP1HIP_TRY(upload(d_progs, flat.data(), flat.size() * 4, s, stage));
         SP1HIP_TRY(upload(d_betas, betas.data(), betas.size() * 16, s, stage));
@@ -972,6 +1050,7 @@
     std::vector<Ext> eval_point(niv + 1);
     for (auto& z : eval_point) z = challenger_sample_ext(ch);
     Ext num_eval = eval_mle_host(out_n, eval_point), den_eval = eval_mle_host(out_d, eval_point);
+    mark("circuit output absorbed");
 
     size_t launch_idx = 0;
     RoundSyncHost rsync;
@@ -1303,7 +1382,9 @@
     }
 
     mark("openings");
+    if (handover) { handover->point = trace_point; handover->openings.assign(openings.begin(), openings.begin() + total_cols); }
     Bytes w;
+    w.b.reserve(need);
     for (const std::vector<Ext>* vv : {&out_n, &out_d}) {
         w.u64(vv->size());
         for (auto& e : *vv) w.ext(e);
@@ -1326,7 +1407,7 @@
         size_t o = 0;
         for (int c = 0; c < n_chips; c++) {
             w.u64(info[c].name.size());
-            for (char chr : info[c].name) w.b.push_back((uint8_t)chr);
+            w.raw(info[c].name.data(), info[c].name.size());
             w.u64(info[c].main_w);
             for (uint32_t k = 0; k < info[c].main_w; k++) w.ext(openings[o + k]);
             w.u64(1); w.u64(info[c].main_w);
@@ -1347,7 +1428,22 @@
     memcpy(h_proof, w.b.data(), w.b.size());
     *proof_len = w.b.size();
     challenger_restore(challenger, ch);
+    mark("proof bytes");
     return SP1HIP_SUCCESS;
 }
 
-}
+namespace sp1hip {
+int logup_gkr_prove_handover(const sp1hip_gkr_chip_t* chips, int n_chips, int max_log_row_count, sp1hip_challenger_t* challenger,
+                             uint8_t* h_proof, size_t* proof_len, sp1hip_stream_t stream, GkrHandover* handover) {
+    return logup_gkr_prove_impl(chips, n_chips, max_log_row_count, challenger, h_proof, proof_len, stream, handover);
+}
+}
+
+extern "C" {
+
+int sp1hip_logup_gkr_prove(const sp1hip_gkr_chip_t* chips, int n_chips, int max_log_row_count, sp1hip_challenger_t* challenger,
+                           uint8_t* h_proof, size_t* proof_len, sp1hip_stream_t stream) {
+    return logup_gkr_prove_impl(chips, n_chips, max_log_row_count, challenger, h_proof, proof_len, stream, nullptr);
+}
+
+}
diff --git a/sp1_amd/csrc/jagged.hip b/sp1_amd/csrc/jagged.hip
--- a/sp1_amd/csrc/jagged.hip
+++ b/sp1_amd/csrc/jagged.hip
@@ -852,6 +852,14 @@
     const bool jg_timing = env_flag("SP1HIP_JG_TIMING", false);
     std::chrono::steady_clock::time_point jg_t[7];
     jg_t[0] = std::chrono::steady_clock::now();
+    std::vector<std::pair<const char*, double>> jg_phases;
+    auto jg_last = jg_t[0];
+    auto jg_mark = [&](const char* what) {
+        if (!jg_timing) return;
+        const auto now = std::chrono::steady_clock::now();
+        jg_phases.emplace_back(what, std::chrono::duration<double, std::milli>(now - jg_last).count());
+        jg_last = now;
+    };
     struct StageMarks {
         bool open = false;
         void next(const char* name) { if (open) roctx_pop(); roctx_push(name); open = true; }
@@ -893,6 +901,7 @@
     }
     const DeviceCtx* ctx;
     SP1HIP_TRY(get_device_ctx(&ctx));
+    jg_mark("shapes and proof size");
 
     JaggedBackend& ch = be;
     SP1HIP_TRY(be.begin());
@@ -912,6 +921,7 @@
     }
     SP1HIP_REQUIRE(column_claims.size() == total_cols, "internal: column claim count");
     const Ext sumcheck_claim = eval_ext_mle_host(column_claims, z_col);
+    jg_mark("z_col sampled, column claims, sumcheck claim");
 
     std::vector<uint32_t> prefix;
     {
@@ -924,9 +934,11 @@
     }
     const uint32_t ncols = (uint32_t)prefix.size() - 1;
     const std::vector<Ext> col_eq = partial_lagrange_host(z_col);
+    jg_mark("prefix sums, eq(z_col)");
 
     Scratch sc;
     SP1HIP_TRY(sc.init(s));
+    jg_mark("scratch, hand-over objects");
     DeviceBuf d_prefix, d_col_eq, d_row_eq;
     SP1HIP_TRY(upload(d_prefix, prefix.data(), prefix.size() * 4, s, sc.stage));
     SP1HIP_TRY(upload(d_col_eq, col_eq.data(), col_eq.size() * 16, s, sc.stage));
@@ -944,6 +956,7 @@
     }
     const JgJ J{d_prefix.u32(), ncols, (const Ext*)d_col_eq.p, d_row_eq.u32(), 1u << max_log_row_count};
     const uint32_t T = segs.total;
+    jg_mark("prefix / eq uploads, row eq table");
 
     marks.next("jagged_sumcheck");
     Sumcheck sumcheck;
@@ -1039,6 +1052,7 @@
     SP1HIP_TRY(tabs[2].alloc((size_t)std::max<uint32_t>((n1 + 1) / 2, 1) * 16, s));
     uint32_t n_live = T;
     int cur = 0;
+    jg_mark("level tables, table descriptors");
     jg_t[1] = std::chrono::steady_clock::now();
     const bool lookahead01 = skip_level1 && !tabs0.empty() && log_m >= 2 && env_flag("SP1HIP_JAGGED_LOOKAHEAD", true);
     for (int round = 0; round < log_m; round++) {
@@ -1176,6 +1190,29 @@
     (void)j_eval;
     const std::vector<Ext>& final_point = sumcheck.point;
 
+    const std::vector<Ext> stack_point(final_point.end() - lsh, final_point.end());
+    hipStream_t* fork_s = nullptr;
+    hipEvent_t* fork_ev = nullptr;
+    SP1HIP_TRY(fork_streams_for(s, 1, &fork_s, &fork_ev));
+    hipStream_t es = fork_s[0];
+    DeviceBuf d_eq;
+    std::vector<DeviceBuf> d_evals(n_rounds);
+    struct Join {
+        hipStream_t st;
+        bool joined = false;
+        ~Join() { if (!joined) (void)hipStreamSynchronize(st); }
+    } fork_join{es};
+    SP1HIP_HIP(hipEventRecord(fork_ev[0], s));
+    SP1HIP_HIP(hipStreamWaitEvent(es, fork_ev[0], 0));
+    SP1HIP_TRY(d_eq.alloc(((size_t)16) << lsh, es));
+    SP1HIP_TRY(sp1hip_partial_lagrange(reinterpret_cast<const sp1hip_ext_t*>(stack_point.data()), lsh, d_eq.u32(), es));
+    for (int r = 0; r < n_rounds; r++) {
+        SP1HIP_TRY(d_evals[r].alloc((size_t)std::max<uint32_t>(round_widths[r], 1) * 16, es));
+        ScopedTimer t("jagged_batch_evals", es);
+        SP1HIP_TRY(sp1hip_mle_eval_columns(rounds[r]->batches.data(), (int)rounds[r]->batches.size(), lsh, d_eq.u32(), d_evals[r].u32(), es));
+    }
+    SP1HIP_HIP(hipEventRecord(fork_ev[1], es));
+
     jg_t[2] = std::chrono::steady_clock::now();
     marks.next("jagged_eval");
     Sumcheck jagged_eval;
@@ -1184,21 +1221,16 @@
     marks.next("stacked_basefold_open");
 
     for (int k = 0; k < 4; k++) ch.observe(q_eval.c[k]);
-    const std::vector<Ext> stack_point(final_point.end() - lsh, final_point.end());
-    DeviceBuf d_eq, d_evals;
-    SP1HIP_TRY(d_eq.alloc(((size_t)16) << lsh, s));
-    SP1HIP_TRY(sp1hip_partial_lagrange(reinterpret_cast<const sp1hip_ext_t*>(stack_point.data()), lsh, d_eq.u32(), stream));
+    SP1HIP_HIP(hipStreamWaitEvent(s, fork_ev[1], 0));
     std::vector<std::vector<Ext>> batch_evals(n_rounds);
     std::vector<Ext> flat_claims;
-    SP1HIP_TRY(d_evals.alloc((size_t)(*std::max_element(round_widths.begin(), round_widths.end())) * 16, s));
     for (int r = 0; r < n_rounds; r++) {
         const uint32_t w = round_widths[r];
         batch_evals[r].resize(w);
-        ScopedTimer t("jagged_batch_evals", s);
-        SP1HIP_TRY(sp1hip_mle_eval_columns(rounds[r]->batches.data(), (int)rounds[r]->batches.size(), lsh, d_eq.u32(), d_evals.u32(), stream));
-        SP1HIP_TRY(sc.mb.fetch(d_evals.p, (size_t)w * 4, batch_evals[r].data()));
+        SP1HIP_TRY(sc.mb.fetch(d_evals[r].p, (size_t)w * 4, batch_evals[r].data()));
         flat_claims.insert(flat_claims.end(), batch_evals[r].begin(), batch_evals[r].end());
     }
+    fork_join.joined = true;
     for (auto& e : flat_claims) for (int k = 0; k < 4; k++) ch.observe(e.c[k]);
     jg_t[4] = std::chrono::steady_clock::now();
     size_t bf_len = need;
@@ -1239,6 +1271,7 @@
         const auto ms = [&](int a, int b) { return std::chrono::duration<double, std::milli>(jg_t[b] - jg_t[a]).count(); };
         fprintf(stderr, "[sp1hip jagged] set-up %.3f ms | %d sumcheck rounds %.3f | jagged-eval %.3f | column evaluations %.3f | BaseFold %.3f | proof bytes %.3f\n",
                 ms(0, 1), log_m, ms(1, 2), ms(2, 3), ms(3, 4), ms(4, 5), ms(5, 6));
+        for (auto& ph : jg_phases) fprintf(stderr, "[sp1hip jagged]   %-44s %8.3f ms\n", ph.first, ph.second);
     }
     return SP1HIP_SUCCESS;
 }
diff --git a/sp1_amd/csrc/shard.hip b/sp1_amd/csrc/shard.hip
--- a/sp1_amd/csrc/shard.hip
+++ b/sp1_amd/csrc/shard.hip
@@ -8,6 +8,7 @@
 
 #include "device_ctx.hpp"
 #include "stacked_data.hpp"
+#include "stage_handover.hpp"
 
 namespace sp1hip {
 void challenger_observe(sp1hip_challenger_t* ch, uint32_t x);
@@ -17,15 +18,6 @@
                          uint64_t total_area, sp1hip_fri_config_t config);
 
 namespace {
-
-struct Reader {
-    const uint8_t* p;
-    size_t n, o = 0;
-    uint64_t u64() { uint64_t v = 0; for (int i = 0; i < 8; i++) v |= (uint64_t)p[o + i] << (8 * i); o += 8; return v; }
-    uint32_t canonical() { uint32_t v = 0; for (int i = 0; i < 4; i++) v |= (uint32_t)p[o + i] << (8 * i); o += 4; return v; }
-    kb::Ext ext() { kb::Ext e; for (int k = 0; k < 4; k++) e.c[k] = kb::to_monty(canonical()); return e; }
-    void skip(size_t k) { o += k; }
-};
 
 void put_u64(std::vector<uint8_t>& b, uint64_t v) { for (int i = 0; i < 8; i++) b.push_back((uint8_t)(v >> (8 * i))); }
 void put_felt(std::vector<uint8_t>& b, uint32_t monty) { const uint32_t v = kb::from_monty(monty); for (int i = 0; i < 4; i++) b.push_back((uint8_t)(v >> (8 * i))); }
@@ -119,6 +111,14 @@
     const bool sh_timing = env_flag("SP1HIP_SHARD_TIMING", false);
     std::chrono::steady_clock::time_point sh_t[6];
     sh_t[0] = std::chrono::steady_clock::now();
+    std::vector<std::pair<const char*, double>> sh_phases;
+    auto sh_last = sh_t[0];
+    auto sh_mark = [&](const char* what) {
+        if (!sh_timing) return;
+        const auto now = std::chrono::steady_clock::now();
+        sh_phases.emplace_back(what, std::chrono::duration<double, std::milli>(now - sh_last).count());
+        sh_last = now;
+    };
     RoctxRange proof_range("sp1hip_prove_shard");
     struct StageMarks {
         hipStream_t s;
@@ -148,6 +148,7 @@
     sp1hip_stacked_data_t* main_data = nullptr;
     SP1HIP_TRY(sp1hip_jagged_commit(tables.data(), n_chips, L, lsh, params.batch_size, params.fri.log_blowup, main_commit, &main_data, stream));
     std::unique_ptr<sp1hip_stacked_data_s> main_guard(main_data);
+    sh_mark("commit (call)");
     for (int k = 0; k < 8; k++) challenger_observe(ch, main_commit[k]);
     challenger_observe(ch, kb::to_monty((uint32_t)n_chips));
     for (int c = 0; c < n_chips; c++) {
@@ -157,39 +158,17 @@
         for (size_t b = 0; b < nl; b++) challenger_observe(ch, kb::to_monty((uint8_t)chips[c].name[b]));
     }
 
+    sh_mark("heights and names observed");
     sh_t[1] = std::chrono::steady_clock::now();
     marks.next("logup_gkr");
     std::vector<uint8_t> gkr_blob(gkr_size);
     size_t glen = gkr_size;
-    SP1HIP_TRY(sp1hip_logup_gkr_prove(gk.data(), n_chips, L, ch, gkr_blob.data(), &glen, stream));
-    std::vector<kb::Ext> zeta(L), openings;
-    {
-        Reader r{gkr_blob.data(), glen};
-        for (int k = 0; k < 2; k++) { const uint64_t m = r.u64(); r.skip(m * 16 + 24); }
-        const uint64_t nr = r.u64();
-        for (uint64_t k = 0; k < nr; k++) {
-            r.skip(64);
-            const uint64_t np = r.u64();
-            for (uint64_t q = 0; q < np; q++) { const uint64_t nc = r.u64(); r.skip(nc * 16); }
-            r.skip(16);
-            const uint64_t pl = r.u64();
-            r.skip(pl * 16 + 16);
-        }
-        SP1HIP_REQUIRE(r.u64() == (uint64_t)L, "internal: GKR point dimension");
-        for (auto& z : zeta) z = r.ext();
-        SP1HIP_REQUIRE(r.u64() == (uint64_t)n_chips, "internal: GKR chip count");
-        for (int c = 0; c < n_chips; c++) {
-            r.skip(r.u64());
-            const uint64_t mw = r.u64();
-            for (uint64_t k = 0; k < mw; k++) openings.push_back(r.ext());
-            r.skip(16);
-            if (r.p[r.o++]) {
-                const uint64_t pw = r.u64();
-                for (uint64_t k = 0; k < pw; k++) openings.push_back(r.ext());
-                r.skip(16);
-            }
-        }
-    }
+    GkrHandover gkr_out;
+    SP1HIP_TRY(logup_gkr_prove_handover(gk.data(), n_chips, L, ch, gkr_blob.data(), &glen, stream, &gkr_out));
+    sh_mark("LogUp-GKR (call)");
+    const std::vector<kb::Ext>& zeta = gkr_out.point;
+    const std::vector<kb::Ext>& openings = gkr_out.openings;
+    SP1HIP_REQUIRE(zeta.size() == (size_t)L && openings.size() == total_w, "internal: GKR hand-over shape");
     sh_t[2] = std::chrono::steady_clock::now();
     marks.next("zerocheck");
     const kb::Ext batching = challenger_sample_ext(ch), gkr_batch = challenger_sample_ext(ch);
@@ -198,34 +177,26 @@
     memcpy(&c_gkr, &gkr_batch, 16);
     std::vector<uint8_t> zc_blob(zc_size);
     size_t zlen = zc_size;
-    SP1HIP_TRY(sp1hip_zerocheck_prove(zc.data(), n_chips, L, reinterpret_cast<const sp1hip_ext_t*>(zeta.data()),
-                                      reinterpret_cast<const sp1hip_ext_t*>(openings.data()), c_batching, c_gkr, h_publics, n_publics, ch,
-                                      zc_blob.data(), &zlen, stream));
-    std::vector<kb::Ext> z_row(L), prep_claims, main_claims;
-    std::vector<std::vector<kb::Ext>> chip_evals(n_chips);
-    {
-        Reader r{zc_blob.data(), zlen};
-        const uint64_t np = r.u64();
-        for (uint64_t q = 0; q < np; q++) { const uint64_t nc = r.u64(); r.skip(nc * 16); }
-        r.skip(16);
-        SP1HIP_REQUIRE(r.u64() == (uint64_t)L, "internal: zerocheck point dimension");
-        for (auto& z : z_row) z = r.ext();
-        r.skip(16);
-        SP1HIP_REQUIRE(r.o == zc_sumcheck_size, "internal: zerocheck sumcheck size");
-        SP1HIP_REQUIRE(r.u64() == (uint64_t)n_chips, "internal: zerocheck chip count");
-        for (int c = 0; c < n_chips; c++) {
-            const uint64_t w = r.u64();
-            SP1HIP_REQUIRE(w == (uint64_t)chips[c].main_width + chips[c].prep_width, "internal: zerocheck opening width");
-            for (uint64_t k = 0; k < w; k++) chip_evals[c].push_back(r.ext());
-            prep_claims.insert(prep_claims.end(), chip_evals[c].begin(), chip_evals[c].begin() + chips[c].prep_width);
-            main_claims.insert(main_claims.end(), chip_evals[c].begin() + chips[c].prep_width, chip_evals[c].end());
-        }
-    }
+    ZcHandover zc_out;
+    SP1HIP_TRY(zerocheck_prove_handover(zc.data(), n_chips, L, reinterpret_cast<const sp1hip_ext_t*>(zeta.data()),
+                                        reinterpret_cast<const sp1hip_ext_t*>(openings.data()), c_batching, c_gkr, h_publics, n_publics, ch,
+                                        zc_blob.data(), &zlen, stream, &zc_out));
+    sh_mark("zerocheck (call)");
+    SP1HIP_REQUIRE(zlen == zc_size && zc_out.point.size() == (size_t)L && zc_out.chip_evals.size() == (size_t)n_chips,
+                   "internal: zerocheck hand-over shape");
+    const std::vector<kb::Ext>& z_row = zc_out.point;
+    const std::vector<std::vector<kb::Ext>>& chip_evals = zc_out.chip_evals;
+    std::vector<kb::Ext> claims;
+    claims.reserve(total_w);
+    for (int c = 0; c < n_chips; c++) {
+        SP1HIP_REQUIRE(chip_evals[c].size() == (size_t)chips[c].main_width + chips[c].prep_width, "internal: zerocheck opening width");
+        claims.insert(claims.end(), chip_evals[c].begin(), chip_evals[c].begin() + chips[c].prep_width);
+    }
+    for (int c = 0; c < n_chips; c++) claims.insert(claims.end(), chip_evals[c].begin() + chips[c].prep_width, chip_evals[c].end());
+    const size_t per_round[2] = {prep_cols, total_w - prep_cols};
+    sh_mark("evaluation proof's claims gathered");
     sh_t[3] = std::chrono::steady_clock::now();
     marks.next("evaluation_proof");
-    std::vector<kb::Ext> claims = prep_claims;
-    claims.insert(claims.end(), main_claims.begin(), main_claims.end());
-    const size_t per_round[2] = {prep_claims.size(), main_claims.size()};
     sp1hip_stacked_data_t* rounds[2] = {preprocessed, main_data};
     SP1HIP_REQUIRE(need >= jag_size, "internal error: shard proof sizes");
     uint8_t* const jag_at = h_proof + (need - jag_size);
@@ -234,6 +205,7 @@
                                    reinterpret_cast<const sp1hip_ext_t*>(claims.data()), per_round, params.fri, ch, jag_at, &jlen,
                                    stream));
     SP1HIP_REQUIRE(jlen == jag_size, "internal error: jagged proof size");
+    sh_mark("evaluation proof (call)");
     (void)s;
 
     sh_t[4] = std::chrono::steady_clock::now();
@@ -272,6 +244,7 @@
         fprintf(stderr, "[sp1hip shard] prologue %.3f ms | commit %.3f | LogUp-GKR %.3f | zerocheck %.3f | evaluation proof %.3f | proof bytes %.3f | %llu arena misses (%.1f MB)\n",
                 std::chrono::duration<double, std::milli>(sh_t[0] - sh_entry).count(), ms(0, 1), ms(1, 2), ms(2, 3), ms(3, 4), ms(4, 5),
                 (unsigned long long)(miss_n1 - miss_n0), (double)(miss_b1 - miss_b0) / 1e6);
+        for (auto& ph : sh_phases) fprintf(stderr, "[sp1hip shard]   %-60s %8.3f ms\n", ph.first, ph.second);
     }
     wait_plan.ok = true;
     return SP1HIP_SUCCESS;
diff --git a/sp1_amd/csrc/stage_handover.hpp b/sp1_amd/csrc/stage_handover.hpp
--- /dev/null
+++ b/sp1_amd/csrc/stage_handover.hpp
@@ -0,0 +1,25 @@
+#pragma once
+#include <vector>
+
+#include "common.hpp"
+#include "kb31.hpp"
+
+namespace sp1hip {
+
+struct GkrHandover {
+    std::vector<kb::Ext> point;
+    std::vector<kb::Ext> openings;
+};
+struct ZcHandover {
+    std::vector<kb::Ext> point;
+    std::vector<std::vector<kb::Ext>> chip_evals;
+};
+
+int logup_gkr_prove_handover(const sp1hip_gkr_chip_t* chips, int n_chips, int max_log_row_count, sp1hip_challenger_t* challenger,
+                             uint8_t* h_proof, size_t* proof_len, sp1hip_stream_t stream, GkrHandover* handover);
+int zerocheck_prove_handover(const sp1hip_zc_chip_t* chips, int n_chips, int max_log_row_count, const sp1hip_ext_t* h_zeta,
+                             const sp1hip_ext_t* h_openings, sp1hip_ext_t alpha, sp1hip_ext_t gkr_batch, const uint32_t* h_publics,
+                             int n_publics, sp1hip_challenger_t* challenger, uint8_t* h_proof, size_t* proof_len,
+                             sp1hip_stream_t stream, ZcHandover* handover);
+
+}
diff --git a/sp1_amd/csrc/zerocheck.hip b/sp1_amd/csrc/zerocheck.hip
--- a/sp1_amd/csrc/zerocheck.hip
+++ b/sp1_amd/csrc/zerocheck.hip
@@ -9,6 +9,7 @@
 
 #include "device_ctx.hpp"
 #include "round_sync.hpp"
+#include "stage_handover.hpp"
 #include "zc_device.hpp"
 #include "zc_poseidon2.hpp"
 #include "zc_keccak.hpp"
@@ -1916,10 +1917,9 @@
 
 struct ByteOut {
     std::vector<uint8_t> b;
-    void u64(uint64_t v) { for (int i = 0; i < 8; i++) b.push_back((uint8_t)(v >> (8 * i))); }
-    void ext(const Ext& e) {
-        for (int k = 0; k < 4; k++) { uint32_t c = kb::from_monty(e.c[k]); for (int i = 0; i < 4; i++) b.push_back((uint8_t)(c >> (8 * i))); }
-    }
+    void raw(const void* src, size_t k) { const uint8_t* p = (const uint8_t*)src; b.insert(b.end(), p, p + k); }
+    void u64(uint64_t v) { raw(&v, 8); }
+    void ext(const Ext& e) { uint32_t v[4]; for (int k = 0; k < 4; k++) v[k] = kb::from_monty(e.c[k]); raw(v, 16); }
 };
 
 }
@@ -1960,7 +1960,7 @@
                                const sp1hip_ext_t* h_zeta, const sp1hip_ext_t* h_openings, sp1hip_ext_t alpha_c,
                                sp1hip_ext_t gkr_c, const uint32_t* h_publics, int n_publics,
                                sp1hip_challenger_t* challenger, uint8_t* h_proof, size_t* proof_len,
-                               sp1hip_stream_t stream) {
+                               sp1hip_stream_t stream, ZcHandover* handover) {
     SP1HIP_REQUIRE(chips && n_chips > 0 && h_zeta && h_openings && challenger && proof_len, "null argument");
     SP1HIP_REQUIRE(max_log_row_count >= 1 && max_log_row_count <= 30, "max_log_row_count out of range");
     SP1HIP_REQUIRE(h_publics || n_publics == 0, "null publics");
@@ -1986,6 +1986,14 @@
     const bool zc_timing = env_flag("SP1HIP_ZC_TIMING", false);
     const auto zc_t0 = std::chrono::steady_clock::now();
     auto zc_t1 = zc_t0, zc_t2 = zc_t0;
+    std::vector<std::pair<const char*, double>> zc_phases;
+    auto zc_last = zc_t0;
+    auto zc_mark = [&](const char* what) {
+        if (!zc_timing) return;
+        const auto now = std::chrono::steady_clock::now();
+        zc_phases.emplace_back(what, std::chrono::duration<double, std::milli>(now - zc_last).count());
+        zc_last = now;
+    };
     const Ext alpha{{alpha_c.c[0], alpha_c.c[1], alpha_c.c[2], alpha_c.c[3]}};
     const Ext gkr{{gkr_c.c[0], gkr_c.c[1], gkr_c.c[2], gkr_c.c[3]}};
     std::vector<uint32_t> publics(h_publics, h_publics + n_publics);
@@ -2004,6 +2012,7 @@
     PinnedStage stage;
     SP1HIP_TRY(stage.init(s));
     if (n_publics) SP1HIP_TRY(stage.upload(d_publics.p, publics.data(), (size_t)n_publics * 4));
+    zc_mark("alpha powers, hand-over objects, publics");
     std::vector<uint32_t> blob;
     Ext rho = kb::ext_zero();
     bool have_rho = false;
@@ -2081,9 +2090,11 @@
         }
         st.push_back(std::move(c));
     }
+    zc_mark("chip plans, claims, program blob");
     DevBuf d_blob;
     SP1HIP_TRY(d_blob.alloc(std::max<size_t>(blob.size(), 4) * 4, s));
     SP1HIP_TRY(stage.upload(d_blob.p, blob.data(), blob.size() * 4));
+    zc_mark("blob upload");
     for (auto& c : st) {
         c->p_prog = d_blob.u32() + c->off_prog;
         c->p_alpha = d_blob.u32() + c->off_alpha;
@@ -2120,6 +2131,7 @@
         SP1HIP_TRY(d_fold[0].alloc(words[0] * 4, s));
         SP1HIP_TRY(d_fold[1].alloc(words[1] * 4, s));
     }
+    zc_mark("eq tables, sums and fold buffers");
     zc_t1 = std::chrono::steady_clock::now();
     auto zc_iter_t = zc_t1;
     double zc_plan_ms = 0, zc_wait_ms = 0, zc_uni_ms = 0;
@@ -2785,6 +2797,7 @@
     update_claims();
     zc_t2 = std::chrono::steady_clock::now();
     ByteOut w;
+    w.b.reserve(need);
     w.u64((uint64_t)L);
     for (auto& m : msgs) { w.u64(m.size()); for (auto& cf : m) w.ext(cf); }
     Ext claimed = kb::ext_zero(), final_eval = kb::ext_zero();
@@ -2835,13 +2848,17 @@
         challenger_observe(challenger, kb::to_monty(wm));
         for (uint32_t k = 0; k < wm; k++) for (int q = 0; q < 4; q++) challenger_observe(challenger, chip_evals[i][wp + k].c[q]);
     }
+    zc_last = zc_t2;
+    zc_mark("opened values fetched, observed, proof bytes");
     if (w.b.size() != need) { set_error("internal error: zerocheck proof size %zu != %zu", w.b.size(), need); return SP1HIP_ERROR_RUNTIME; }
     memcpy(h_proof, w.b.data(), need);
     *proof_len = need;
+    if (handover) { handover->point = point; handover->chip_evals = std::move(chip_evals); }
     if (zc_timing) {
         const auto ms = [](std::chrono::steady_clock::time_point a, std::chrono::steady_clock::time_point b) { return std::chrono::duration<double, std::milli>(b - a).count(); };
         fprintf(stderr, "[sp1hip zerocheck] set-up %.3f ms | %d rounds %.3f ms (planning + launches %.3f, waiting for the sums %.3f, univariates + transcript %.3f) | openings + proof %.3f ms\n",
                 ms(zc_t0, zc_t1), L, ms(zc_t1, zc_t2), zc_plan_ms, zc_wait_ms, zc_uni_ms, ms(zc_t2, std::chrono::steady_clock::now()));
+        for (auto& ph : zc_phases) fprintf(stderr, "[sp1hip zerocheck]   %-44s %8.3f ms\n", ph.first, ph.second);
     }
     return SP1HIP_SUCCESS;
 }
@@ -2984,8 +3001,16 @@
     sp1hip_challenger_t* backup = nullptr;
     if (challenger) SP1HIP_TRY(sp1hip_challenger_clone(challenger, &backup));
     const int st = zerocheck_prove_impl(chips, n_chips, max_log_row_count, h_zeta, h_openings, alpha, gkr_batch, h_publics,
-                                        n_publics, challenger, h_proof, proof_len, stream);
+                                        n_publics, challenger, h_proof, proof_len, stream, nullptr);
     if (st != SP1HIP_SUCCESS && challenger) challenger_restore(challenger, backup);
     sp1hip_challenger_free(backup);
     return st;
 }
+
+int sp1hip::zerocheck_prove_handover(const sp1hip_zc_chip_t* chips, int n_chips, int max_log_row_count, const sp1hip_ext_t* h_zeta,
+                                     const sp1hip_ext_t* h_openings, sp1hip_ext_t alpha, sp1hip_ext_t gkr_batch,
+                                     const uint32_t* h_publics, int n_publics, sp1hip_challenger_t* challenger, uint8_t* h_proof,
+                                     size_t* proof_len, sp1hip_stream_t stream, ZcHandover* handover) {
+    return zerocheck_prove_impl(chips, n_chips, max_log_row_count, h_zeta, h_openings, alpha, gkr_batch, h_publics, n_publics,
+                                challenger, h_proof, proof_len, stream, handover);
+}
```

Result: slower. 96.17 million (-1.4%).
